# charles-kmc/Semi-blind-image-deblurring-problems-with-TV

Hardware: AMD Instinct MI355X
Metric: SALSA outer-iters/sec + final PSNR, 2048x2048 Gaussian blur (higher is better)
Workload: dtype f64; 1 GPU; SALSA_v2 TV deblur, one 2048x2048 image per GPU, Gaussian PSF 7x7, BSNR 30 dB, TViters=10; images_per_gpu=1, parallelism=images x1

## Files before the change

semi-blind-image-deblurring-problems-with-tv_amd/csrc/ctx.hip:

```cpp
#include <chrono>
#include <cmath>
#include <cstring>
#include <algorithm>
#include <mutex>
#include <thread>
#include <vector>

#include "sbtv_internal.h"

namespace sbtv {

static std::string g_error;
static std::mutex g_error_mu;

void set_global_error(const std::string &msg) {
    std::lock_guard<std::mutex> lk(g_error_mu);
    g_error = msg;
}

int fail(sbtv_ctx *ctx, int code, const std::string &msg) {
    if (ctx) ctx->err = msg;
    set_global_error(msg);
    return code;
}
// ... 348 lines not shown
    const int rc = init();
    if (rc != 0) {
        const std::string msg = ctx->err;
        (void)sbtv_ctx_destroy(ctx);
        return fail(nullptr, rc, msg);
    }
    *out = ctx;
    return 0;
}

int sbtv_ctx_destroy(sbtv_ctx *ctx) {
    if (!ctx) return 0;
    if (ctx->lanes) (void)sbtv_group_destroy(ctx->lanes);
    ctx->lanes = nullptr;
    (void)hipSetDevice(ctx->device);
    if (ctx->stream) (void)hipStreamSynchronize(ctx->stream);
    for (auto &kv : ctx->ws)
        if (kv.second.base) (void)hipFree(kv.second.base);
    if (ctx->canary_desc) (void)hipFree(ctx->canary_desc);
    if (ctx->canary_bad) (void)hipFree(ctx->canary_bad);
    for (auto &kv : ctx->twiddles) (void)hipFree(kv.second);
    for (auto &kv : ctx->any_axes) (void)hipFree(kv.second);
    if (ctx->pinned) (void)hipHostFree(ctx->pinned);
    for (auto &l : ctx->stage) {
        for (int k = 0; k < 2; ++k) {
            if (l.pin[k]) (void)hipHostFree(l.pin[k]);
            if (l.ev[k]) (void)hipEventDestroy(l.ev[k]);
        }
        if (l.s) (void)hipStreamDestroy(l.s);
    }
    for (auto &ev : ctx->ev)
        if (ev) (void)hipEventDestroy(ev);
    for (auto &ev : ctx->loop_ev)
        if (ev) (void)hipEventDestroy(ev);
    if (ctx->own_stream && ctx->stream) (void)hipStreamDestroy(ctx->stream);
    delete ctx;
    return 0;
}

int sbtv_ctx_set_stream(sbtv_ctx *ctx, void *hip_stream) {
    if (!ctx) return SBTV_ERR_BADARG;
    SBTV_HIP(ctx, hipSetDevice(ctx->device));
    SBTV_HIP(ctx, hipStreamSynchronize(ctx->stream));
    if (hip_stream == nullptr) {
        if (!ctx->own_stream) {
            SBTV_HIP(ctx, hipStreamCreateWithFlags(&ctx->stream, hipStreamNonBlocking));
            ctx->own_stream = true;
        }
        return 0;
    }
    if (ctx->own_stream && ctx->stream) SBTV_HIP(ctx, hipStreamDestroy(ctx->stream));
    ctx->stream = (hipStream_t)hip_stream;
    ctx->own_stream = false;
    return 0;
}

int sbtv_ctx_sync(sbtv_ctx *ctx) {
    if (!ctx) return SBTV_ERR_BADARG;
    SBTV_HIP(ctx, hipStreamSynchronize(ctx->stream));
    return 0;
}

int sbtv_callcounter_get(const sbtv_ctx *ctx, long long *calls) {
    if (!ctx || !calls) return SBTV_ERR_BADARG;
    *calls = ctx->calls;
    return 0;
}

int sbtv_callcounter_reset(sbtv_ctx *ctx) {
    if (!ctx) return SBTV_ERR_BADARG;
    ctx->calls = 0;
    return 0;
}

int sbtv_last_timing(const sbtv_ctx *ctx, double out[4]) {
    if (!ctx || !out) return SBTV_ERR_BADARG;
    for (int i = 0; i < 4; ++i) out[i] = ctx->timing[i];
    return 0;
}

int sbtv_last_host_stats(const sbtv_ctx *ctx, double out[14]) {
    if (!ctx || !out) return SBTV_ERR_BADARG;
    const HostStats &h = ctx->hstat;
    const double v[14] = {h.waits, h.ready_at_once, h.waits_slept, h.sleeps, h.stream_queries,
                          h.wait_s, h.wait_max_s, h.enqueue_s, h.enqueue_max_s, h.wait_max_outer,
                          h.nvcsw, h.nivcsw, h.minflt, h.majflt};
    for (int i = 0; i < 14; ++i) out[i] = v[i];
    return 0;
}

int sbtv_host_transpose(const double *src, double *dst, int batch, int rows, int cols) {
    if (!src || !dst || batch < 0 || rows < 0 || cols < 0) return SBTV_ERR_BADARG;
    constexpr int BS = 64;
    const long long nbr = ((long long)rows + BS - 1) / BS;
    const long long jobs = nbr * batch;
    auto work = [&](int t, int T) {
        for (long long job = t; job < jobs; job += T) {
            const int b = (int)(job / nbr), r0 = (int)(job % nbr) * BS, r1 = std::min(rows, r0 + BS);
            const double *s = src + (size_t)b * rows * cols;
            double *d = dst + (size_t)b * rows * cols;
            for (int c0 = 0; c0 < cols; c0 += BS) {
                const int c1 = std::min(cols, c0 + BS);
                for (int c = c0; c < c1; ++c)
                    for (int r = r0; r < r1; ++r) d[(size_t)c * rows + r] = s[(size_t)r * cols + c];
            }
        }
    };
    const size_t bytes = (size_t)batch * rows * cols * sizeof(double);
    const int T = bytes >= ((size_t)4 << 20) ? 4 : 1;
    std::vector<std::thread> th;
    int started = 1;
    try {
        for (int t = 1; t < T; ++t, ++started) th.emplace_back(work, t, T);
    } catch (...) {
    }
    work(0, T);
    for (auto &x : th) x.join();
    for (int t = started; t < T; ++t) work(t, T);
    return 0;
}

int sbtv_diag_solve_stats(const sbtv_ctx *ctx, double out[4]) {
    if (!ctx || !out) return SBTV_ERR_BADARG;
    for (int i = 0; i < 4; ++i) out[i] = ctx->solve_stats[i];
    if (ctx->lanes)
        for (int r = 0; r < sbtv_group_size(ctx->lanes); ++r)
            for (int i = 0; i < 4; ++i) out[i] += sbtv_group_ctx(ctx->lanes, r)->solve_stats[i];
    return 0;
}

int sbtv_diag_stage_stats(const sbtv_ctx *ctx, double out[4]) {
    if (!ctx || !out) return SBTV_ERR_BADARG;
    for (int i = 0; i < 4; ++i) out[i] = ctx->stage_stats[i];
    if (ctx->lanes)
        for (int r = 0; r < sbtv_group_size(ctx->lanes); ++r)
            for (int i = 0; i < 4; ++i) out[i] += sbtv_group_ctx(ctx->lanes, r)->stage_stats[i];
    return 0;
}

int sbtv_diag_workspace(sbtv_ctx *ctx, const char *name, void **dptr, size_t *bytes) {
    if (!ctx || !name || !dptr) return SBTV_ERR_BADARG;
    auto it = ctx->ws.find(name);
    if (it == ctx->ws.end() || !it->second.p) return fail(ctx, SBTV_ERR_BADARG, std::string("no workspace named '") + name + "'");
    *dptr = it->second.p;
    if (bytes) *bytes = it->second.bytes;
    return 0;
}

int sbtv_diag_switches(char *buf, size_t cap) {
    static const char *const names[] = {
        "SBTV_CANARY", "SBTV_COLLECT_RIDE", "SBTV_EXACT", "SBTV_FFT_WAVE", "SBTV_FISTA_FUSED_STEP", "SBTV_FISTA_LAG",
        "SBTV_FUSED_VARIANT", "SBTV_GRAPH", "SBTV_INLINE_CTRL", "SBTV_PROX_SPEC", "SBTV_SAPG_DEFER",
        "SBTV_SAPG_FUSED_MYULA", "SBTV_SAPG_HOST", "SBTV_SINGLE_STEP", "SBTV_SPIN", "SBTV_TAG_SPIN_US", "SBTV_TILE_ORDER", "SBTV_SALSA_NOX", "SBTV_CSALSA_SPECTRAL",
        "SBTV_CORAL_BATCH", "SBTV_ROWS_FOLD", "SBTV_ERR_SUBSET", "SBTV_LANES", "SBTV_LANE_COUNT", "SBTV_STAGE_THREADS", "SBTV_TEST_FAIL_SAPG", "SBTV_FUSED_STAGGER"};
    if (!buf || cap == 0) return SBTV_ERR_BADARG;
    std::string s;
    int nset = 0;
    for (const char *n : names)
        if (const char *e = getenv(n)) {
            s += (nset++ ? " " : "");
            s += n;
            s += "=";
            s += e;
        }
    if (s.size() + 1 > cap) s.resize(cap - 1);
    memcpy(buf, s.c_str(), s.size() + 1);
    return nset;
}

int sbtv_diag_canary(sbtv_ctx *ctx, int poke, int *enabled, int *nbuf, int *nbad) {
    if (!ctx) return SBTV_ERR_BADARG;
    SBTV_HIP(ctx, hipSetDevice(ctx->device));
    if (enabled) *enabled = ctx->canary ? 1 : 0;
    int nb = 0, bad = 0;
    if (ctx->canary && poke) {
        for (auto &kv : ctx->ws)
            if (kv.second.base) {
                SBTV_HIP(ctx, hipMemsetAsync(static_cast<unsigned char *>(kv.second.p) + kv.second.bytes, 0, 8, ctx->stream));
                break;
            }
    }
    std::string name;
    SBTV_TRY(canary_verify(ctx, &nb, &bad, &name));
    if (ctx->canary && poke && bad) {
        for (auto &kv : ctx->ws)
            if (kv.second.base) {
                SBTV_HIP(ctx, hipMemsetAsync(static_cast<unsigned char *>(kv.second.p) + kv.second.bytes, kGuardByte, kGuard, ctx->stream));
                break;
            }
        SBTV_HIP(ctx, hipStreamSynchronize(ctx->stream));
    }
    if (nbuf) *nbuf = nb;
    if (nbad) *nbad = bad;
    return 0;
}

int sbtv_malloc(sbtv_ctx *ctx, size_t bytes, void **dptr) {
    if (!ctx || !dptr) return SBTV_ERR_BADARG;
    SBTV_HIP(ctx, hipSetDevice(ctx->device));
    SBTV_HIP(ctx, hipMalloc(dptr, bytes));
    return 0;
}

int sbtv_free(sbtv_ctx *ctx, void *dptr) {
    if (!ctx) return SBTV_ERR_BADARG;
    SBTV_HIP(ctx, hipStreamSynchronize(ctx->stream));
    SBTV_HIP(ctx, hipFree(dptr));
    return 0;
}

int sbtv_memcpy_h2d(sbtv_ctx *ctx, void *dst, const void *src, size_t bytes) {
    if (!ctx) return SBTV_ERR_BADARG;
    SBTV_HIP(ctx, hipSetDevice(ctx->device));
    if (stage_threaded(bytes)) {
        SBTV_HIP(ctx, hipStreamSynchronize(ctx->stream));
        return stage_copy(ctx, dst, src, bytes, true);
    }
    SBTV_HIP(ctx, hipMemcpyAsync(dst, src, bytes, hipMemcpyHostToDevice, ctx->stream));
    SBTV_HIP(ctx, hipStreamSynchronize(ctx->stream));
    return 0;
}

int sbtv_memcpy_d2h(sbtv_ctx *ctx, void *dst, const void *src, size_t bytes) {
    if (!ctx) return SBTV_ERR_BADARG;
    SBTV_HIP(ctx, hipSetDevice(ctx->device));
    if (stage_threaded(bytes)) {
        SBTV_HIP(ctx, hipStreamSynchronize(ctx->stream));
        return stage_copy(ctx, dst, src, bytes, false);
    }
    SBTV_HIP(ctx, hipMemcpyAsync(dst, src, bytes, hipMemcpyDeviceToHost, ctx->stream));
    SBTV_HIP(ctx, hipStreamSynchronize(ctx->stream));
    return 0;
}

static double spectral_norm_sq(const double *D, int t) {
    double B[15 * 15];
    for (int i = 0; i < t; ++i)
        for (int j = 0; j < t; ++j) {
            double s = 0.0;
            for (int k = 0; k < t; ++k) s += D[i * t + k] * D[j * t + k];
            B[i * t + j] = s;
        }
    for (int sweep = 0; sweep < 60; ++sweep) {
        double off = 0.0, diag = 0.0;
        for (int i = 0; i < t; ++i)
            for (int j = 0; j < t; ++j) (i == j ? diag : off) += B[i * t + j] * B[i * t + j];
        if (off <= 1e-34 * diag || off == 0.0) break;
        for (int p = 0; p < t - 1; ++p)
            for (int q = p + 1; q < t; ++q) {
                const double apq = B[p * t + q];
                if (apq == 0.0) continue;
                const double theta = (B[q * t + q] - B[p * t + p]) / (2.0 * apq);
                const double tt = (theta >= 0 ? 1.0 : -1.0) / (fabs(theta) + sqrt(theta * theta + 1.0));
                const double cs = 1.0 / sqrt(tt * tt + 1.0), sn = tt * cs;
                for (int k = 0; k < t; ++k) {
                    const double bkp = B[k * t + p], bkq = B[k * t + q];
                    B[k * t + p] = cs * bkp - sn * bkq;
                    B[k * t + q] = sn * bkp + cs * bkq;
                }
                for (int k = 0; k < t; ++k) {
                    const double bpk = B[p * t + k], bqk = B[q * t + k];
                    B[p * t + k] = cs * bpk - sn * bqk;
                    B[q * t + k] = sn * bpk + cs * bqk;
                }
            }
    }
    double mx = 0.0;
    for (int i = 0; i < t; ++i) mx = fmax(mx, B[i * t + i]);
    return mx;
}

int sbtv_err_psf(int kind, int taille, const double *ps, int n, const double *p_true, double phi, double *out) {
    if (kind < 0 || kind > 2 || taille < 1 || taille > 15 || !ps || !p_true || !out || n < 1)
        return fail(nullptr, SBTV_ERR_PSF, "sbtv_err_psf: bad arguments");
    const int t2 = taille * taille;
    double truth[225], cur[225], D[225];
    double pt[3] = {p_true[0], kind == SBTV_PSF_LAPLACE ? 0.0 : p_true[1], kind == SBTV_PSF_GAUSSIAN ? phi : 0.0};
    int rc = sbtv_psf_taps(kind, taille, pt, truth, nullptr, nullptr);
    if (rc != 0) return rc;
    for (int i = 0; i < n; ++i) {
        if (kind == SBTV_PSF_MOFFAT && i == 0) {
            out[0] = 0.0;
            continue;
        }
        double p[3] = {ps[i], 0.0, kind == SBTV_PSF_GAUSSIAN ? phi : 0.0};
        if (kind == SBTV_PSF_GAUSSIAN) p[1] = ps[n + (i > 0 ? i - 1 : 0)];
        if (kind == SBTV_PSF_MOFFAT) p[1] = ps[n + i];
        rc = sbtv_psf_taps(kind, taille, p, cur, nullptr, nullptr);
        if (rc != 0) return rc;
        for (int q = 0; q < t2; ++q) D[q] = cur[q] - truth[q];
        out[i] = spectral_norm_sq(D, taille);
    }
    return 0;
}

int sbtv_psf_taps(int kind, int taille, const double *p, double *taps, double *d0, double *d1) {
    if (taille < 1 || taille > 15 || !p || !taps)
        return fail(nullptr, SBTV_ERR_PSF, "sbtv_psf_taps: bad arguments (1 <= taille <= 15)");
    const int t = taille;
    if (kind != SBTV_PSF_GAUSSIAN && kind != SBTV_PSF_MOFFAT && kind != SBTV_PSF_LAPLACE)
        return fail(nullptr, SBTV_ERR_PSF, "sbtv_psf_taps: unknown PSF kind");
    std::vector<double> f(t * t), e0(t * t, 0.0), e1(t * t, 0.0);
    double s = 0, s0 = 0, s1 = 0;
    for (int q = 0; q < t * t; ++q) psf_taps_point(kind, t, p, q, &f[q], &e0[q], &e1[q]);
    for (int q = 0; q < t * t; ++q) { s += f[q]; s0 += e0[q]; s1 += e1[q]; }
    for (int q = 0; q < t * t; ++q) {
        taps[q] = f[q] / s;
// ... 8 lines not shown
```

semi-blind-image-deblurring-problems-with-tv_amd/csrc/elementwise.hip:

```cpp
#include "sbtv_internal.h"

#pragma clang fp contract(off)

namespace sbtv {

constexpr int EWB = 256;

__device__ __forceinline__ double ew_wave_sum(double v) {
#pragma unroll
    for (int off = 32; off > 0; off >>= 1) v += __shfl_xor(v, off, 64);
    return v;
}

template <int NQ>
__device__ __forceinline__ void ew_block_sum(double (&v)[NQ], double *red ) {
    const int lane = threadIdx.x & 63, w = threadIdx.x >> 6;
#pragma unroll
    for (int c = 0; c < NQ; ++c) {
        const double a = ew_wave_sum(v[c]);
        if (lane == 0) red[c * 4 + w] = a;
    }
    __syncthreads();
    if (threadIdx.x == 0) {
#pragma unroll
        for (int c = 0; c < NQ; ++c) v[c] = (red[c * 4] + red[c * 4 + 1]) + (red[c * 4 + 2] + red[c * 4 + 3]);
    }
}

int ew_blocks(size_t P) {
    size_t nb = (P / 2 + EWB - 1) / EWB;
    if (nb > 1024) nb = 1024;
    if (nb < 1) nb = 1;
    return (int)nb;
}

__global__ __launch_bounds__(EWB) void salsa_zero_start_kernel(const double *__restrict__ y, const double *__restrict__ tru,
                                                                double *__restrict__ x, double *__restrict__ u,
                                                                double *__restrict__ bu, double *__restrict__ accp,
                                                                double *__restrict__ postp, size_t P, double scale) {
    const int b = blockIdx.y;
    __shared__ double red[2 * 4];
    const size_t base = (size_t)b * P;
    double acc[2] = {0, 0};
    for (size_t q = (size_t)blockIdx.x * EWB + threadIdx.x; q < P; q += (size_t)gridDim.x * EWB) {
        const double yv = y[base + q];
        const double tv = tru ? tru[base + q] : 0.0;
        acc[0] += yv * yv;
        acc[1] += tv * tv;
        x[base + q] = 0.0;
        u[base + q] = 0.0;
        bu[base + q] = 0.0;
    }
    ew_block_sum<2>(acc, red);
    if (threadIdx.x == 0) {
        const size_t G = gridDim.x;
        for (int q = 0; q < 3; ++q) accp[((size_t)b * 3 + q) * G + blockIdx.x] = (q == 0) ? acc[0] * scale : 0.0;
        for (int q = 0; q < 6; ++q) postp[((size_t)b * 6 + q) * G + blockIdx.x] = (q == 0) ? acc[1] : 0.0;
    }
}

__global__ __launch_bounds__(EWB) void pair_sums_kernel(const double *__restrict__ a, const double *__restrict__ c,
                                                         double *__restrict__ partials, size_t P) {
    const int b = blockIdx.y;
    __shared__ double red[3 * 4];
    __shared__ double redm[4];
    const size_t base = (size_t)b * P;
    double acc[3] = {0, 0, 0};
    double mx = -1.0e308;
    for (size_t q = (size_t)blockIdx.x * EWB + threadIdx.x; q < P; q += (size_t)gridDim.x * EWB) {
        const double av = a[base + q];
        const double cv = c ? c[base + q] : 0.0;
        const double d = av - cv;
        acc[0] += d * d;
        acc[1] += av * av;
        acc[2] += cv * cv;
        mx = fmax(mx, av);
    }
    for (int off = 32; off > 0; off >>= 1) mx = fmax(mx, __shfl_xor(mx, off, 64));
    if ((threadIdx.x & 63) == 0) redm[threadIdx.x >> 6] = mx;
    ew_block_sum<3>(acc, red);
    if (threadIdx.x == 0) {
        for (int q = 0; q < 3; ++q) partials[((size_t)b * 4 + q) * gridDim.x + blockIdx.x] = acc[q];
        partials[((size_t)b * 4 + 3) * gridDim.x + blockIdx.x] = fmax(fmax(redm[0], redm[1]), fmax(redm[2], redm[3]));
    }
}

__global__ __launch_bounds__(256) void reduce_max_kernel(const double *__restrict__ partials, int n,
                                                          double *__restrict__ out) {
    __shared__ double redm[4];
    const double *p = partials + (size_t)blockIdx.x * n;
    double mx = -1.0e308;
    for (int q = threadIdx.x; q < n; q += 256) mx = fmax(mx, p[q]);
    for (int off = 32; off > 0; off >>= 1) mx = fmax(mx, __shfl_xor(mx, off, 64));
    if ((threadIdx.x & 63) == 0) redm[threadIdx.x >> 6] = mx;
    __syncthreads();
    if (threadIdx.x == 0) out[blockIdx.x] = fmax(fmax(redm[0], redm[1]), fmax(redm[2], redm[3]));
}

__global__ __launch_bounds__(EWB) void axpy_kernel(double *__restrict__ y, const double *__restrict__ gr, double a,
                                                    size_t Ptot, ProxArm arm, int batch) {
    if (arm.ctrl && blockIdx.x == 0 && (int)threadIdx.x < batch) {
        const int b = threadIdx.x;
        ProxCtrl c = arm.ctrl[b];
        c.k = 0;
        c.done = (arm.frozen && arm.frozen[b]) ? 1 : 0;
        c.cur = 0;
        c.maxiter = arm.maxiter;
        c.redo = 0;
        c.f_valid = 0;
        c.err = 0.0;
        c.lambda = arm.lambda[b];
        c.tol = arm.tol;
        c.tau = arm.tau;
        arm.ctrl[b] = c;
    }
    for (size_t q = (size_t)blockIdx.x * EWB + threadIdx.x; q < Ptot / 2; q += (size_t)gridDim.x * EWB) {
        double2 yv = *reinterpret_cast<double2 *>(y + 2 * q);
        const double2 gv = *reinterpret_cast<const double2 *>(gr + 2 * q);
        yv.x = yv.x - a * gv.x;
        yv.y = yv.y - a * gv.y;
        *reinterpret_cast<double2 *>(y + 2 * q) = yv;
    }
}
__global__ __launch_bounds__(EWB) void fista_momentum_kernel(const double *__restrict__ x, const double *__restrict__ xold,
                                                              double *__restrict__ y, const double *__restrict__ tru,
                                                              double c, double *__restrict__ partials, size_t P,
                                                              const int *__restrict__ frozen) {
    const int b = blockIdx.y;
    if (frozen && frozen[b]) return;
    __shared__ double red[3 * 4];
    const size_t base = (size_t)b * P;
    double acc[3] = {0, 0, 0};
    for (size_t q = (size_t)blockIdx.x * EWB + threadIdx.x; q < P / 2; q += (size_t)gridDim.x * EWB) {
        const size_t o = base + 2 * q;
        const double2 xv = *reinterpret_cast<const double2 *>(x + o);
        const double2 xo = *reinterpret_cast<const double2 *>(xold + o);
        const double d0 = xv.x - xo.x, d1 = xv.y - xo.y;
        *reinterpret_cast<double2 *>(y + o) = make_double2(xv.x + c * d0, xv.y + c * d1);
        if (tru) {
            const double2 tv = *reinterpret_cast<const double2 *>(tru + o);
            const double e0 = xv.x - tv.x, e1 = xv.y - tv.y;
            acc[0] += e0 * e0 + e1 * e1;
        }
        acc[1] += d0 * d0 + d1 * d1;
        acc[2] += xv.x * xv.x + xv.y * xv.y;
    }
    ew_block_sum<3>(acc, red);
    if (threadIdx.x == 0)
        for (int q = 0; q < 3; ++q) partials[((size_t)b * 3 + q) * gridDim.x + blockIdx.x] = acc[q];
}

template <bool MOM>
__global__ __launch_bounds__(EWB) void myula_step_kernel(double *__restrict__ X, const double *__restrict__ prox,
                                                          const double *__restrict__ grad,
                                                          const double *__restrict__ Z,
                                                          const double *__restrict__ sigma2, double gam, double lamb,
                                                          double sq2g, size_t P, RngArgs rng, ProxArm arm, MomArgs mom) {
    const int b = blockIdx.y;
    if (arm.ctrl && blockIdx.x == 0 && threadIdx.x == 0) {
        ProxCtrl c = arm.ctrl[b];
        c.k = 0;
        c.done = 0;
        c.cur = 0;
        c.maxiter = arm.maxiter;
        c.redo = 0;
        c.f_valid = 0;
        c.err = 0.0;
        c.lambda = arm.lambda[b];
        c.tol = arm.tol;
        c.tau = arm.tau;
        arm.ctrl[b] = c;
    }
    const size_t base = (size_t)b * P;
    const double s2 = sigma2[b];
    const unsigned step = rng.step_dev ? (unsigned)rng.step_dev[0] : rng.step;
    const int k = MOM ? mom_sample(mom) : 0;
    const double rk = 1.0 / (double)(k > 0 ? k : 1);
    for (size_t q = (size_t)blockIdx.x * EWB + threadIdx.x; q < P / 2; q += (size_t)gridDim.x * EWB) {
        const size_t o = base + 2 * q;
        const double2 xv = *reinterpret_cast<const double2 *>(X + o);
        const double2 pv = *reinterpret_cast<const double2 *>(prox + o);
        const double2 gv = *reinterpret_cast<const double2 *>(grad + o);
        const double2 zv = Z ? *reinterpret_cast<const double2 *>(Z + o)
                             : philox_normal_pair(q, step, rng.chain0 + (unsigned)b, rng.seed);
        double2 r;
        r.x = myula_nocontract(xv.x, pv.x, gv.x, 1.0, zv.x, gam, lamb, s2, sq2g);
        r.y = myula_nocontract(xv.y, pv.y, gv.y, 1.0, zv.y, gam, lamb, s2, sq2g);
        *reinterpret_cast<double2 *>(X + o) = r;
        if (MOM && k > 0) moments_pair(mom, o, r, k, rk);
    }
}

template <bool MOM>
__global__ __launch_bounds__(EWB) void myula_plain_kernel(double *__restrict__ X, const double *__restrict__ prox,
                                                           const double *__restrict__ grad,
                                                           const double *__restrict__ Z,
                                                           const double *__restrict__ sigma2, double gam, double lamb,
                                                           double sq2g, size_t P, RngArgs rng, ProxArm arm, MomArgs mom) {
    const int b = blockIdx.y;
    if (arm.ctrl && blockIdx.x == 0 && threadIdx.x == 0) {
        ProxCtrl c = arm.ctrl[b];
        c.k = 0;
        c.done = 0;
        c.cur = 0;
        c.maxiter = arm.maxiter;
        c.redo = 0;
        c.f_valid = 0;
        c.err = 0.0;
        c.lambda = arm.lambda[b];
        c.tol = arm.tol;
        c.tau = arm.tau;
        arm.ctrl[b] = c;
    }
    const size_t base = (size_t)b * P;
    const double s2 = sigma2[b], keep = 1.0 - gam / lamb;
    const int k = MOM ? mom_sample(mom) : 0;
    const double rk = 1.0 / (double)(k > 0 ? k : 1);
    for (size_t q = (size_t)blockIdx.x * EWB + threadIdx.x; q < P / 2; q += (size_t)gridDim.x * EWB) {
        const size_t o = base + 2 * q;
        const double2 xv = *reinterpret_cast<const double2 *>(X + o);
        const double2 pv = *reinterpret_cast<const double2 *>(prox + o);
        const double2 gv = *reinterpret_cast<const double2 *>(grad + o);
        const double2 zv = Z ? *reinterpret_cast<const double2 *>(Z + o)
                             : philox_normal_pair(q, rng.step, rng.chain0 + (unsigned)b, rng.seed);
        double2 r;
        r.x = (keep * xv.x - gam * (gv.x / s2 - pv.x / lamb)) + sq2g * zv.x;
        r.y = (keep * xv.y - gam * (gv.y / s2 - pv.y / lamb)) + sq2g * zv.y;
        *reinterpret_cast<double2 *>(X + o) = r;
        if (MOM && k > 0) moments_pair(mom, o, r, k, rk);
    }
}

__global__ __launch_bounds__(EWB) void moments_seed_kernel(const double *__restrict__ X, double *__restrict__ mean,
                                                           double *__restrict__ m2, size_t n2) {
    const MomArgs m{mean, m2, 1, nullptr, 1, 1};
    for (size_t q = (size_t)blockIdx.x * EWB + threadIdx.x; q < n2; q += (size_t)gridDim.x * EWB)
        moments_pair(m, 2 * q, *reinterpret_cast<const double2 *>(X + 2 * q), 1, 1.0);
}

__global__ __launch_bounds__(EWB) void moments_finish_kernel(const double *__restrict__ mean, const double *__restrict__ m2,
                                                             size_t P, int batch, double n, int pooled, int raw,
                                                             double *__restrict__ mean_out, double *__restrict__ var_out) {
#pragma clang fp contract(off)
    const int b = blockIdx.y;
    for (size_t i = (size_t)blockIdx.x * EWB + threadIdx.x; i < P; i += (size_t)gridDim.x * EWB) {
        double mu = mean[(size_t)b * P + i], s = m2[(size_t)b * P + i], na = n;
        if (pooled) {
            for (int c = 1; c < batch; ++c) {
                const double mb = mean[(size_t)c * P + i], sb = m2[(size_t)c * P + i];
                const double nt = na + n, d = mb - mu;
                mu = mu + d * (n / nt);
                s = (s + sb) + d * d * (na * n / nt);
                na = nt;
            }
        }
        mean_out[(size_t)b * P + i] = mu;
        if (var_out) var_out[(size_t)b * P + i] = raw ? s : (na > 1.0 ? s / (na - 1.0) : 0.0);
    }
}

int myula_plain_step(sbtv_ctx *ctx, double *X, const double *prox, const double *grad, const double *Z,
                     const double *sigma2_dev, double gam, double lamb, size_t P, int batch, const RngArgs *rng,
                     const ProxArm *arm, const MomArgs *mom) {
    if (!Z && !rng) return fail(ctx, SBTV_ERR_BADARG, "myula_plain_step: neither a noise array nor generator arguments");
    const RngArgs r = rng ? *rng : RngArgs{0ull, 0u, 0u, nullptr};
    const ProxArm pa = arm ? *arm : ProxArm{nullptr, nullptr, 0, 0.0, 0.0, nullptr};
    if (mom)
        hipLaunchKernelGGL(myula_plain_kernel<true>, dim3(ew_blocks(P), batch), dim3(EWB), 0, ctx->stream, X, prox, grad, Z,
                           sigma2_dev, gam, lamb, sqrt(2 * gam), P, r, pa, *mom);
    else
        hipLaunchKernelGGL(myula_plain_kernel<false>, dim3(ew_blocks(P), batch), dim3(EWB), 0, ctx->stream, X, prox, grad, Z,
                           sigma2_dev, gam, lamb, sqrt(2 * gam), P, r, pa, MomArgs{});
    SBTV_HIP(ctx, hipGetLastError());
    return 0;
}

int moments_seed(sbtv_ctx *ctx, const double *X, double *mean, double *m2, size_t P, int batch) {
    const size_t n = P * batch;
    hipLaunchKernelGGL(moments_seed_kernel, dim3(ew_blocks(n)), dim3(EWB), 0, ctx->stream, X, mean, m2, n / 2);
    SBTV_HIP(ctx, hipGetLastError());
    return 0;
}

int moments_finish(sbtv_ctx *ctx, const double *mean, const double *m2, size_t P, int batch, long long n, const MomReq &req) {
    const int pooled = req.pooled && !req.raw;
    const size_t nout = P * (pooled ? 1 : batch);
    double *mo = nullptr, *vo = nullptr;
    const int fl = req.dev ? SBTV_DEVICE_PTRS : SBTV_HOST_PTRS;
    SBTV_TRY(stage_out_buf(ctx, "mom.mean_out", req.mean, nout, fl, &mo));
    if (req.var) SBTV_TRY(stage_out_buf(ctx, "mom.var_out", req.var, nout, fl, &vo));
    hipLaunchKernelGGL(moments_finish_kernel, dim3(ew_blocks(2 * P), pooled ? 1 : batch), dim3(EWB), 0, ctx->stream, mean,
                       m2, P, batch, (double)n, pooled, req.raw ? 1 : 0, mo, vo);
    SBTV_HIP(ctx, hipGetLastError());
    SBTV_TRY(stage_out_copy(ctx, req.mean, mo, nout, fl));
    if (req.var) SBTV_TRY(stage_out_copy(ctx, req.var, vo, nout, fl));
    if (req.count)
        for (size_t c = 0; c < (pooled ? 1 : (size_t)batch); ++c) req.count[c] = pooled ? n * batch : n;
    return 0;
}

int pair_sums(sbtv_ctx *ctx, const double *a, const double *c, size_t P, int batch, double *out4_dev) {
    const int nb = ew_blocks(P);
    double *partials = nullptr;
    SBTV_TRY(ws_get_t(ctx, "ew.pair.partials", (size_t)batch * 4 * nb, &partials));
    hipLaunchKernelGGL(pair_sums_kernel, dim3(nb, batch), dim3(EWB), 0, ctx->stream, a, c, partials, P);
    SBTV_HIP(ctx, hipGetLastError());
    for (int b = 0; b < batch; ++b) {
        SBTV_TRY(reduce_partials(ctx, partials + (size_t)b * 4 * nb, 3, nb, out4_dev + (size_t)b * 4));
        hipLaunchKernelGGL(reduce_max_kernel, dim3(1), dim3(256), 0, ctx->stream, partials + ((size_t)b * 4 + 3) * nb,
                           nb, out4_dev + (size_t)b * 4 + 3);
    }
    SBTV_HIP(ctx, hipGetLastError());
    return 0;
}

int salsa_zero_start(sbtv_ctx *ctx, const double *y, const double *tru, double *x, double *u, double *bu, size_t P, int batch,
                     double scale, double **accp, double **postp, int *nblk) {
    const int G = ew_blocks(2 * P);
    SBTV_TRY(ws_get_t(ctx, "ew.zero.acc", (size_t)batch * 3 * G, accp));
    SBTV_TRY(ws_get_t(ctx, "ew.zero.post", (size_t)batch * 6 * G, postp));
    hipLaunchKernelGGL(salsa_zero_start_kernel, dim3(G, batch), dim3(EWB), 0, ctx->stream, y, tru, x, u, bu, *accp, *postp, P,
                       scale);
    SBTV_HIP(ctx, hipGetLastError());
    *nblk = G;
    return 0;
}

int axpy(sbtv_ctx *ctx, double *y, const double *gr, double a, size_t Ptot, const ProxArm *arm, int batch) {
    if (arm && batch > EWB) return fail(ctx, SBTV_ERR_BADARG, "axpy: cannot arm more than 256 control blocks");
    const ProxArm pa = arm ? *arm : ProxArm{nullptr, nullptr, 0, 0.0, 0.0, nullptr};
    hipLaunchKernelGGL(axpy_kernel, dim3(ew_blocks(Ptot)), dim3(EWB), 0, ctx->stream, y, gr, a, Ptot, pa, batch);
    SBTV_HIP(ctx, hipGetLastError());
    return 0;
}

int fista_momentum(sbtv_ctx *ctx, const double *x, const double *xold, double *y, const double *tru, double coef,
                   double *partials, size_t P, int batch, const int *frozen) {
    hipLaunchKernelGGL(fista_momentum_kernel, dim3(ew_blocks(P), batch), dim3(EWB), 0, ctx->stream, x, xold, y, tru,
                       coef, partials, P, frozen);
    SBTV_HIP(ctx, hipGetLastError());
    return 0;
}

int myula_step(sbtv_ctx *ctx, double *X, const double *prox, const double *grad, const double *Z,
               const double *sigma2_dev, double gam, double lamb, size_t P, int batch, const RngArgs *rng,
               const ProxArm *arm, const MomArgs *mom) {
    if (!Z && !rng) return fail(ctx, SBTV_ERR_BADARG, "myula_step: neither a noise array nor generator arguments");
    const RngArgs r = rng ? *rng : RngArgs{0ull, 0u, 0u, nullptr};
    const ProxArm pa = arm ? *arm : ProxArm{nullptr, nullptr, 0, 0.0, 0.0, nullptr};
    if (mom)
        hipLaunchKernelGGL(myula_step_kernel<true>, dim3(ew_blocks(P), batch), dim3(EWB), 0, ctx->stream, X, prox, grad, Z,
                           sigma2_dev, gam, lamb, sqrt(2 * gam), P, r, pa, *mom);
    else
        hipLaunchKernelGGL(myula_step_kernel<false>, dim3(ew_blocks(P), batch), dim3(EWB), 0, ctx->stream, X, prox, grad, Z,
                           sigma2_dev, gam, lamb, sqrt(2 * gam), P, r, pa, MomArgs{});
    SBTV_HIP(ctx, hipGetLastError());
    return 0;
}

}

using namespace sbtv;

extern "C" {

static int metric_common(sbtv_ctx *ctx, const double *x_true, const double *x, int M, int N, int batch, double *out,
                         int flags, bool psnr) {
    if (!ctx) return SBTV_ERR_BADARG;
    if (!x_true || !x || !out || M < 1 || N < 1 || batch < 1) return fail(ctx, SBTV_ERR_BADARG, "metric: bad arguments");
    SBTV_HIP(ctx, hipSetDevice(ctx->device));
    const size_t P = (size_t)M * N;
    const double *a = nullptr, *c = nullptr;
    SBTV_TRY(stage_in(ctx, "metric.a", x_true, P * batch, flags, &a));
    SBTV_TRY(stage_in(ctx, "metric.c", x, P * batch, flags, &c));
    double *o4 = nullptr;
    SBTV_TRY(ws_get_t(ctx, "metric.out", (size_t)batch * 4, &o4));
    SBTV_TRY(pair_sums(ctx, a, c, P, batch, o4));
    std::vector<double> h((size_t)batch * 4);
    SBTV_HIP(ctx, hipMemcpyAsync(h.data(), o4, sizeof(double) * batch * 4, hipMemcpyDeviceToHost, ctx->stream));
    SBTV_HIP(ctx, hipStreamSynchronize(ctx->stream));
    for (int b = 0; b < batch; ++b) {
        const double se = h[(size_t)b * 4], mx = h[(size_t)b * 4 + 3];
        if (psnr)
            out[b] = 10 * log10(mx * mx) - 10 * log10(se / (double)P);
        else
            out[b] = 10 * log10(se / (double)P);
    }
    return canary_epilogue(ctx, 0);
}

int sbtv_PSNR(sbtv_ctx *ctx, const double *x_true, const double *x, int M, int N, int batch, double *out, int flags) {
    return metric_common(ctx, x_true, x, M, N, batch, out, flags, true);
}
int sbtv_MSE(sbtv_ctx *ctx, const double *x_true, const double *x, int M, int N, int batch, double *out, int flags) {
    return metric_common(ctx, x_true, x, M, N, batch, out, flags, false);
}

}
```

semi-blind-image-deblurring-problems-with-tv_amd/csrc/fft.hip:

```cpp
#include <type_traits>

#include "sbtv_internal.h"

namespace sbtv {

__device__ __forceinline__ double2 cadd(double2 a, double2 b) { return make_double2(a.x + b.x, a.y + b.y); }
__device__ __forceinline__ double2 csub(double2 a, double2 b) { return make_double2(a.x - b.x, a.y - b.y); }
__device__ __forceinline__ double2 cmul(double2 a, double2 b) {
    return make_double2(a.x * b.x - a.y * b.y, a.x * b.y + a.y * b.x);
}
__device__ __forceinline__ double2 cmulc(double2 a, double2 b) {
    return make_double2(a.x * b.x + a.y * b.y, a.y * b.x - a.x * b.y);
}
__device__ __forceinline__ double2 cconj(double2 a) { return make_double2(a.x, -a.y); }
__device__ __forceinline__ double2 cscale(double2 a, double s) { return make_double2(a.x * s, a.y * s); }
__device__ __forceinline__ double cabs2(double2 a) { return a.x * a.x + a.y * a.y; }

constexpr int TWS = 2;
constexpr int TW = 1 << TWS;
__device__ __forceinline__ size_t s_tiled(int k, int l, int n1) {
    return (((size_t)(l >> TWS) * n1 + k) << TWS) + (l & (TW - 1));
}
__device__ __forceinline__ size_t u_tiled(int k, int l, int n1) { return ((size_t)(l >> TWS) * (n1 + 1) + k) * TW + (l & (TW - 1)); }

// ... 264 lines not shown
        double2 r;
        if (e == 0) {
            r = make_double2(Z.x + Z.y, Z.x - Z.y);
        } else {
            const double2 w = tw_M[e];
            const double2 su = cadd(Z, Zm), di = csub(Z, Zm);
            const double2 wd = cmul(w, di);
            r = make_double2(0.5 * (su.x + wd.y), 0.5 * (su.y - wd.x));
        }
        out[e] = r;
    }
}

typedef double sbtv_d2 __attribute__((ext_vector_type(2)));
__device__ __forceinline__ double2 nt_load2(const double *p) {
    const sbtv_d2 v = __builtin_nontemporal_load(reinterpret_cast<const sbtv_d2 *>(p));
    return make_double2(v.x, v.y);
}
__device__ __forceinline__ void nt_store2(double *p, double2 v) {
    sbtv_d2 w;
    w.x = v.x;
    w.y = v.y;
    __builtin_nontemporal_store(w, reinterpret_cast<sbtv_d2 *>(p));
}
template <int LOG2N, bool POST>
__global__ __launch_bounds__(COLS_THREADS) void fft_cols_inv_kernel(const double2 *__restrict__ S,
                                                                     double *__restrict__ x,
                                                                     const double2 *__restrict__ tw_n1,
                                                                     const double2 *__restrict__ tw_M, int N,
                                                                     double scale, const int *__restrict__ frozen,
                                                                     ColsPost post) {
    constexpr int n = 1 << LOG2N, T = n / 8;
    constexpr int LDSN = n + (n >> 3);
    constexpr int MAXSEQ = (COLS_THREADS / T) > 0 ? (COLS_THREADS / T) : 1;
    __shared__ double lds[2 * MAXSEQ * LDSN];
    const int b = blockIdx.y;
    if (frozen && frozen[b]) return;
    const int nseq = blockDim.x / T;
    const int seq = threadIdx.x / T, t = threadIdx.x - seq * T;
    const int j = blockIdx.x * nseq + seq;
    const size_t colbase = ((size_t)b * N + j) * n;
    const double2 *__restrict__ in = S + colbase;
    ColsX X{lds + seq * LDSN, MAXSEQ * LDSN};
    double2 v[8], m[8];
#pragma unroll
    for (int s = 0; s < 8; ++s) v[s] = in[t + s * T];
    constexpr bool PREP = POST && (LOG2N <= 8);
    double2 pu[PREP ? 8 : 1], pb[PREP ? 8 : 1], pt[PREP ? 8 : 1], pul[PREP ? 8 : 1], pxo[PREP ? 8 : 1];
    double pup[PREP ? 8 : 1];
    if constexpr (PREP) {
        constexpr int M = 2 * n;
        const size_t ibase = (size_t)b * N * M, cb = ibase + (size_t)j * M;
        const size_t cl = ibase + (size_t)(j > 0 ? j - 1 : N - 1) * M;
#pragma unroll
        for (int s = 0; s < 8; ++s) {
            const int e = t + s * T;
            const size_t o = cb + 2 * (size_t)e;
            pu[s] = *reinterpret_cast<const double2 *>(post.u + o);
            pb[s] = *reinterpret_cast<const double2 *>(post.bu + o);
            if (post.tru) pt[s] = nt_load2(post.tru + o);
            if (post.xprev) pxo[s] = *reinterpret_cast<const double2 *>(post.xprev + o);
            pup[s] = post.u[e > 0 ? o - 1 : cb + M - 1];
            pul[s] = *reinterpret_cast<const double2 *>(post.u + cl + 2 * (size_t)e);
        }
    }
    mirror<LOG2N>(v, m, t, X);
#pragma unroll
    for (int s = 0; s < 8; ++s) {
        const int e = t + s * T;
        if (e == 0) {
            const double X0 = v[s].x, Xn = v[s].y;
            v[s] = make_double2(0.5 * (X0 + Xn), 0.5 * (X0 - Xn));
        } else {
            const double2 Xk = v[s], Xm = cconj(m[s]);
            const double2 E = cscale(cadd(Xk, Xm), 0.5);
            const double2 O = cmulc(cscale(csub(Xk, Xm), 0.5), tw_M[e]);
            v[s] = make_double2(E.x - O.y, E.y + O.x);
        }
    }
    fft_stages<LOG2N, 0, true>(v, t, tw_n1, X);
    double2 *__restrict__ out = reinterpret_cast<double2 *>(x) + colbase;
    if constexpr (!POST) {
#pragma unroll
        for (int s = 0; s < 8; ++s) out[t + s * T] = cscale(v[s], scale);
    } else {
        constexpr int M = 2 * n;
        const size_t ibase = (size_t)b * N * M;
        const size_t cb = ibase + (size_t)j * M;
        const size_t cl = ibase + (size_t)(j > 0 ? j - 1 : N - 1) * M;
        double acc[6] = {0.0, 0.0, 0.0, 0.0, 0.0, 0.0};
#pragma unroll
        for (int s = 0; s < 8; ++s) {
            const int e = t + s * T;
            const size_t o = cb + 2 * (size_t)e;
            const double2 xv = cscale(v[s], scale);
            nt_store2(reinterpret_cast<double *>(out + e), xv);
            const double2 uv = PREP ? pu[PREP ? s : 0] : *reinterpret_cast<const double2 *>(post.u + o);
            double2 bv = PREP ? pb[PREP ? s : 0] : *reinterpret_cast<const double2 *>(post.bu + o);
            bv.x = bv.x + (uv.x - xv.x);
            bv.y = bv.y + (uv.y - xv.y);
            *reinterpret_cast<double2 *>(post.bu + o) = bv;
            *reinterpret_cast<double2 *>(post.g + o) = make_double2(xv.x - bv.x, xv.y - bv.y);
            if (post.tru) {
                const double2 tv = PREP ? pt[PREP ? s : 0] : nt_load2(post.tru + o);
                const double e0 = xv.x - tv.x, e1 = xv.y - tv.y;
                acc[0] += e0 * e0 + e1 * e1;
            }
            const double d0 = xv.x - uv.x, d1 = xv.y - uv.y;
            acc[1] += d0 * d0 + d1 * d1;
            acc[2] += xv.x * xv.x + xv.y * xv.y;
            acc[3] += uv.x * uv.x + uv.y * uv.y;
            if (post.xprev) {
                const double2 xo = PREP ? pxo[PREP ? s : 0] : *reinterpret_cast<const double2 *>(post.xprev + o);
                const double p0 = xv.x - xo.x, p1 = xv.y - xo.y;
                acc[4] += p0 * p0 + p1 * p1;
            }
            const double up = PREP ? pup[PREP ? s : 0] : post.u[e > 0 ? o - 1 : cb + M - 1];
            const double2 ul = PREP ? pul[PREP ? s : 0] : *reinterpret_cast<const double2 *>(post.u + cl + 2 * (size_t)e);
            const double h0 = uv.x - ul.x, v0 = uv.x - up, h1 = uv.y - ul.y, v1 = uv.y - uv.x;
            acc[5] += sqrt(h0 * h0 + v0 * v0) + sqrt(h1 * h1 + v1 * v1);
        }
        __syncthreads();
        const int nthr = blockDim.x;
#pragma unroll
        for (int c = 0; c < 6; ++c) lds[c * nthr + threadIdx.x] = acc[c];
        __syncthreads();
        for (int stride = nthr >> 1; stride > 0; stride >>= 1) {
            if ((int)threadIdx.x < stride) {
#pragma unroll
                for (int c = 0; c < 6; ++c) lds[c * nthr + threadIdx.x] += lds[c * nthr + threadIdx.x + stride];
            }
            __syncthreads();
        }
        if (threadIdx.x < 6) post.partials[((size_t)b * 6 + threadIdx.x) * gridDim.x + blockIdx.x] = lds[threadIdx.x * nthr];
    }
}

struct RowsParams {
    const double2 *Sin;
    double2 *Sout;
    const double2 *tw;
    const double2 *H, *Y, *D1, *D2;
    double2 *E;
    const double *cs;
    const double *mu;
    double *acc;
    const int *frozen;
    int n1;
    int fwd, inv, op;
    int shared_spec;
    int fold;
    size_t u_img;
    int u_tiled;
};

template <int OP>
__device__ __forceinline__ double2 spec_apply(double2 V, double2 H, double2 Y, double2 D1, double2 D2, double mu,
                                              double wgt, double (&acc)[3]) {
    if constexpr (OP == OP_MUL_H) {
        return cmul(V, H);
    } else if constexpr (OP == OP_MUL_HC) {
        return cmulc(V, H);
    } else if constexpr (OP == OP_INVLS) {
        const double d = cabs2(H) + mu;
        return make_double2(V.x / d, V.y / d);
    } else if constexpr (OP == OP_ATA) {
        return cscale(V, cabs2(H));
    } else if constexpr (OP == OP_SALSA) {
        const double d = cabs2(H) + mu;
        const double2 num = cadd(cmulc(Y, H), cscale(V, mu));
#ifdef SBTV_SPEC_IEEE_DIV
        const double rd = 1.0 / d;
#else
        const double rd = fast_rcp(d);
#endif
        const double2 Xh = make_double2(num.x * rd, num.y * rd);
        const double2 R = csub(Y, cmul(H, Xh));
        acc[0] += wgt * cabs2(R);
        return Xh;
    } else if constexpr (OP == OP_RESID) {
        const double2 R = csub(cmul(H, V), Y);
        acc[0] += wgt * cabs2(R);
        return V;
    } else if constexpr (OP == OP_GRADF) {
        const double2 R = csub(cmul(H, V), Y);
        acc[0] += wgt * cabs2(R);
        return cmulc(R, H);
    } else if constexpr (OP == OP_GRAD) {
        const double2 R = csub(cmul(H, V), Y);
        acc[0] += wgt * cabs2(R);
        const double2 d1 = cmulc(cmul(D1, V), R), d2 = cmulc(cmul(D2, V), R);
        acc[1] += wgt * d1.x;
        acc[2] += wgt * d2.x;
        return cmulc(R, H);
    } else {
        return V;
    }
}

struct CsPar {
    double c_y, c_e, c_keep;
};
__device__ __forceinline__ double2 spec_apply_cs(double2 V, double2 H, double2 Y, double2 &E, double mu, const CsPar &c,
                                                 double wgt, double (&acc)[3]) {
    const double d = cabs2(H) + mu;
    const double2 W = cadd(cscale(Y, c.c_y), cscale(E, c.c_e));
    const double2 num = cadd(cmulc(W, H), cscale(V, mu));
#ifdef SBTV_SPEC_IEEE_DIV
    const double rd = 1.0 / d;
#else
    const double rd = fast_rcp(d);
#endif
    const double2 Xh = make_double2(num.x * rd, num.y * rd);
    const double2 T = csub(cmul(H, Xh), Y);
    const double2 En = cadd(T, cscale(E, c.c_keep));
    acc[0] += wgt * cabs2(T);
    acc[1] += wgt * cabs2(En);
    acc[2] += wgt * cabs2(csub(En, E));
    E = En;
    return Xh;
}

template <int LOG2N, int RK, int OP>
__global__ __launch_bounds__(RK *((1 << LOG2N) / 8), 1) void fft_rows_kernel(RowsParams p) {
    constexpr int N = 1 << LOG2N, T = N / 8;
    constexpr int LDSI = RK * N;
    constexpr int LDSN = LDSI + ((LDSI >> 5) << 2) + 8;
    __shared__ double lds[2 * LDSN];
    __shared__ double red[3 * 16];
    const int b = blockIdx.y;
    if (p.frozen && p.frozen[b]) return;
    const int q = threadIdx.x % RK, t = threadIdx.x / RK;
    int kb;
    {
        const int nt = gridDim.x, bid = blockIdx.x;
        const int q8 = nt >> 3, r8 = nt & 7, x = bid & 7, o = bid >> 3;
        kb = (x < r8 ? x * (q8 + 1) : r8 * (q8 + 1) + (x - r8) * q8) + o;
    }
    const int k = kb * RK + q;
    const int n1 = p.n1;
    const size_t ibase = (size_t)b * n1 * N;
    const double2 *__restrict__ in = p.Sin + ibase;
    RowsX<RK> X{lds, LDSN, q};
    double2 v[8];
    auto sidx = [&](int l) -> size_t { return (size_t)l * n1 + k; };
    auto uidx = [&](int kk, int l) -> size_t { return (size_t)l * (p.n1 + 1) + kk; };
#pragma unroll
    for (int s = 0; s < 8; ++s) v[s] = in[sidx(t + s * T)];
    constexpr bool CS = (OP == OP_CSALSA);
    constexpr bool PRE = (OP != OP_NONE) && !CS && (RK * T <= 256);
    constexpr bool needY = (OP == OP_SALSA || OP == OP_RESID || OP == OP_GRAD || OP == OP_GRADF || CS);
    constexpr bool needD = (OP == OP_GRAD);
    const size_t hbase = p.shared_spec ? 0 : (size_t)b * p.u_img;
    double2 hh[PRE ? 8 : 1], yy[(PRE && needY) ? 8 : 1], dd1[(PRE && needD) ? 8 : 1], dd2[(PRE && needD) ? 8 : 1];
    double2 hq[PRE ? 8 : 1], yq[(PRE && needY) ? 8 : 1], d1q[(PRE && needD) ? 8 : 1], d2q[(PRE && needD) ? 8 : 1];
    if constexpr (PRE) {
#pragma unroll
        for (int s = 0; s < 8; ++s) {
            const size_t hi = hbase + uidx(k, t + s * T);
            hh[s] = p.H[hi];
            if constexpr (needY) yy[s] = p.Y[hi];
            if constexpr (needD) {
                dd1[s] = p.D1[hi];
                dd2[s] = p.D2[hi];
            }
        }
        if (kb == 0 && q == 0) {
#pragma unroll
            for (int s = 0; s < 8; ++s) {
                const size_t hn = hbase + uidx(n1, t + s * T);
                hq[s] = p.H[hn];
                if constexpr (needY) yq[s] = p.Y[hn];
                if constexpr (needD) {
                    d1q[s] = p.D1[hn];
                    d2q[s] = p.D2[hn];
                }
            }
        }
    }
    if (p.fwd) fft_stages<LOG2N, 0, false>(v, t, p.tw, X);

    double acc[3] = {0.0, 0.0, 0.0};
    if constexpr (OP != OP_NONE) {
        const double mu = p.mu ? p.mu[b] : 0.0;
        if constexpr (CS) {
            const CsPar cp{p.cs[0], p.cs[1], p.cs[2]};
            double2 *__restrict__ Ep = p.E + hbase;
            const double2 *__restrict__ Hp = p.H + hbase, *__restrict__ Yp = p.Y + hbase;
            if (kb == 0) {
                double2 m[8];
                mirror<LOG2N>(v, m, t, X);
#pragma unroll
                for (int s = 0; s < 8; ++s) {
                    const int l = t + s * T;
                    if (q == 0) {
                        const size_t h0 = uidx(0, l), hn = uidx(n1, l);
                        const double2 P = v[s], Q = cconj(m[s]);
                        const double2 A = cscale(cadd(P, Q), 0.5);
                        const double2 dB = csub(P, Q);
                        const double2 B = make_double2(0.5 * dB.y, -0.5 * dB.x);
                        double2 e0 = Ep[h0], en = Ep[hn];
                        const double2 A2 = spec_apply_cs(A, Hp[h0], Yp[h0], e0, mu, cp, 1.0, acc);
                        const double2 B2 = spec_apply_cs(B, Hp[hn], Yp[hn], en, mu, cp, 1.0, acc);
                        Ep[h0] = e0;
                        Ep[hn] = en;
                        v[s] = make_double2(A2.x - B2.y, A2.y + B2.x);
// ... 261 lines not shown
    const PassDims cd = cols_dims(pl);
    hipLaunchKernelGGL((fft_cols_inv_kernel<L, false>), dim3(cd.wgs, pl.batch), dim3(cd.threads), 0,
                       ctx->stream, S, x, pl.tw_n1, pl.tw_M, pl.N, scale, frozen, ColsPost{});
}
template <int L>
static void launch_cols_inv_post(sbtv_ctx *ctx, const FftPlan &pl, const double2 *S, double *x, double scale,
                                 const int *frozen, const ColsPost &post) {
    const PassDims cd = cols_dims(pl);
    hipLaunchKernelGGL((fft_cols_inv_kernel<L, true>), dim3(cd.wgs, pl.batch), dim3(cd.threads), 0,
                       ctx->stream, S, x, pl.tw_n1, pl.tw_M, pl.N, scale, frozen, post);
}

#define SBTV_DISPATCH_LOG2(L, CALL)                                    \
    switch (L) {                                                       \
        case 3: CALL(3); break;                                        \
        case 4: CALL(4); break;                                        \
        case 5: CALL(5); break;                                        \
        case 6: CALL(6); break;                                        \
        case 7: CALL(7); break;                                        \
        case 8: CALL(8); break;                                        \
        case 9: CALL(9); break;                                        \
        case 10: CALL(10); break;                                      \
        case 11: CALL(11); break;                                      \
        default: return fail(ctx, SBTV_ERR_SIZE, "unsupported FFT length"); \
    }

bool fft_cols_tv_ok(const FftPlan &pl) { return !pl.generic; }
int fft_cols_fwd_f(sbtv_ctx *ctx, const FftPlan &pl, const double *x, const double *add, double2 *S,
                   const int *frozen, double *tvp) {
    if (tvp && (!fft_cols_tv_ok(pl) || add)) return fail(ctx, SBTV_ERR_BADARG, "fft_cols_fwd: TV partials not available for this call");
    if (pl.generic) return any_cols_fwd(ctx, pl, x, add, S, frozen);
    if (pl.wave) {
        const PassDims cd = cols_dims(pl);
        const dim3 grid(cd.wgs, pl.batch), block(cd.threads);
        if (pl.n1 == 1024)
            hipLaunchKernelGGL((cols_fwd_wave_kernel<10, 16>), grid, block, 0, ctx->stream, x, add, S, pl.tw_n1, pl.tw_M,
                               pl.N, frozen, tvp);
        else
            hipLaunchKernelGGL((cols_fwd_wave_kernel<9, 8>), grid, block, 0, ctx->stream, x, add, S, pl.tw_n1, pl.tw_M,
                               pl.N, frozen, tvp);
        SBTV_HIP(ctx, hipGetLastError());
        return 0;
    }
    const int L = ilog2(pl.n1);
#define CALL(LL) launch_cols_fwd<LL>(ctx, pl, x, add, S, frozen, tvp)
    SBTV_DISPATCH_LOG2(L, CALL)
#undef CALL
    SBTV_HIP(ctx, hipGetLastError());
    return 0;
}
int fft_cols_fwd(sbtv_ctx *ctx, const FftPlan &pl, const double *x, const double *add, double2 *S) {
    return fft_cols_fwd_f(ctx, pl, x, add, S, nullptr, nullptr);
}

int fft_cols_inv_f(sbtv_ctx *ctx, const FftPlan &pl, const double2 *S, double *x, double scale, const int *frozen) {
    if (pl.generic) return any_cols_inv(ctx, pl, S, x, scale, frozen, nullptr);
    if (pl.wave) {
        const PassDims cd = cols_dims(pl);
        const dim3 grid(cd.wgs, pl.batch), block(cd.threads);
        if (pl.n1 == 1024)
            hipLaunchKernelGGL((cols_inv_wave_kernel<10, 16, 0>), grid, block, 0, ctx->stream, S, x, pl.tw_n1,
                               pl.tw_M, pl.N, scale, frozen, ColsPost{});
        else
            hipLaunchKernelGGL((cols_inv_wave_kernel<9, 8, 0>), grid, block, 0, ctx->stream, S, x, pl.tw_n1, pl.tw_M,
                               pl.N, scale, frozen, ColsPost{});
        SBTV_HIP(ctx, hipGetLastError());
        return 0;
    }
    const int L = ilog2(pl.n1);
#define CALL(LL) launch_cols_inv<LL>(ctx, pl, S, x, scale, frozen)
    SBTV_DISPATCH_LOG2(L, CALL)
#undef CALL
    SBTV_HIP(ctx, hipGetLastError());
    return 0;
}
bool fft_cols_inv_step_ok(const FftPlan &pl) { return !pl.generic && pl.wave; }
static int fft_cols_step_check(sbtv_ctx *ctx, const FftPlan &pl, const char *who) {
    if (!fft_cols_inv_step_ok(pl)) return fail(ctx, SBTV_ERR_BADARG, std::string(who) + ": size not on the wave-granular path");
    return 0;
}
int fft_cols_inv_step(sbtv_ctx *ctx, const FftPlan &pl, const double2 *S, double *y, double scale, double alpha,
                      const int *frozen) {
    SBTV_TRY(fft_cols_step_check(ctx, pl, "fft_cols_inv_step"));
    ColsPost post;
    post.ystep = y;
    post.alpha = alpha;
    const PassDims cd = cols_dims(pl);
        const dim3 grid(cd.wgs, pl.batch), block(cd.threads);
    if (pl.n1 == 1024)
        hipLaunchKernelGGL((cols_inv_wave_kernel<10, 16, 8>), grid, block, 0, ctx->stream, S, (double *)nullptr, pl.tw_n1,
                           pl.tw_M, pl.N, scale, frozen, post);
    else
        hipLaunchKernelGGL((cols_inv_wave_kernel<9, 8, 8>), grid, block, 0, ctx->stream, S, (double *)nullptr, pl.tw_n1, pl.tw_M,
                           pl.N, scale, frozen, post);
    SBTV_HIP(ctx, hipGetLastError());
    return 0;
}
int fft_cols_inv_sub(sbtv_ctx *ctx, const FftPlan &pl, const double2 *S, double *x, double scale, const double *b, double *g) {
    SBTV_TRY(fft_cols_step_check(ctx, pl, "fft_cols_inv_sub"));
    ColsPost post;
    post.bu_in = b;
    post.g = g;
    const PassDims cd = cols_dims(pl);
        const dim3 grid(cd.wgs, pl.batch), block(cd.threads);
    if (pl.n1 == 1024)
        hipLaunchKernelGGL((cols_inv_wave_kernel<10, 16, 64>), grid, block, 0, ctx->stream, S, x, pl.tw_n1, pl.tw_M, pl.N, scale,
                           (const int *)nullptr, post);
    else
        hipLaunchKernelGGL((cols_inv_wave_kernel<9, 8, 64>), grid, block, 0, ctx->stream, S, x, pl.tw_n1, pl.tw_M, pl.N, scale,
                           (const int *)nullptr, post);
    SBTV_HIP(ctx, hipGetLastError());
    return 0;
}
int fft_cols_inv_myula(sbtv_ctx *ctx, const FftPlan &pl, const double2 *S, double scale, double *X, const double *prox,
                       const double *Z, const double *sigma2_dev, double gam, double lamb, const RngArgs *rng,
                       const ProxArm *arm, const MomArgs *mom) {
    SBTV_TRY(fft_cols_step_check(ctx, pl, "fft_cols_inv_myula"));
    if (!Z && !rng) return fail(ctx, SBTV_ERR_BADARG, "fft_cols_inv_myula: neither a noise array nor generator arguments");
    ColsPost post;
    post.ystep = X;
    post.mprox = prox;
    post.mZ = Z;
    post.msig2 = sigma2_dev;
    post.mgam = gam;
    post.mlamb = lamb;
    post.msq2g = sqrt(2 * gam);
    if (rng) post.mrng = *rng;
    if (arm) post.marm = *arm;
    const PassDims cd = cols_dims(pl);
        const dim3 grid(cd.wgs, pl.batch), block(cd.threads);
    if (mom) {
        post.mom = *mom;
        if (pl.n1 == 1024)
            hipLaunchKernelGGL((cols_inv_wave_kernel<10, 16, 16 | 128>), grid, block, 0, ctx->stream, S, (double *)nullptr,
                               pl.tw_n1, pl.tw_M, pl.N, scale, (const int *)nullptr, post);
        else
            hipLaunchKernelGGL((cols_inv_wave_kernel<9, 8, 16 | 128>), grid, block, 0, ctx->stream, S, (double *)nullptr,
                               pl.tw_n1, pl.tw_M, pl.N, scale, (const int *)nullptr, post);
    } else if (pl.n1 == 1024)
        hipLaunchKernelGGL((cols_inv_wave_kernel<10, 16, 16>), grid, block, 0, ctx->stream, S, (double *)nullptr, pl.tw_n1,
                           pl.tw_M, pl.N, scale, (const int *)nullptr, post);
    else
        hipLaunchKernelGGL((cols_inv_wave_kernel<9, 8, 16>), grid, block, 0, ctx->stream, S, (double *)nullptr, pl.tw_n1, pl.tw_M,
                           pl.N, scale, (const int *)nullptr, post);
    SBTV_HIP(ctx, hipGetLastError());
    return 0;
}
int fft_cols_inv(sbtv_ctx *ctx, const FftPlan &pl, const double2 *S, double *x, double scale) {
    return fft_cols_inv_f(ctx, pl, S, x, scale, nullptr);
}
int fft_cols_blocks(const FftPlan &pl) { return (pl.wave || pl.generic) ? pl.N : pl.N / cols_nseq(pl); }
int fft_cols_inv_post(sbtv_ctx *ctx, const FftPlan &pl, const double2 *S, double *x, double scale, const int *frozen,
                      const ColsPost &post) {
    if ((!pl.wave && (post.bu_in || post.skip_x)) || (post.bu_in && !post.skip_x))
        return fail(ctx, SBTV_ERR_BADARG, "fft_cols_inv_post: bu_in + skip_x go together and need the wave-granular column pass");
    if (pl.generic) return any_cols_inv(ctx, pl, S, x, scale, frozen, &post);
    if (pl.wave) {
        const PassDims cd = cols_dims(pl);
        const dim3 grid(cd.wgs, pl.batch), block(cd.threads);
        if (post.skip_x && (!post.bu_in || post.bu_in == post.bu || post.xprev))
            return fail(ctx, SBTV_ERR_BADARG, "fft_cols_inv_post: skip_x needs a separate bu_in and no xprev");
        const int pm = 1 + (post.tru ? 2 : 0) + (post.xprev ? 4 : 0) + (post.skip_x ? 32 : 0);
#define SBTV_POST_CASE(PM_)                                                                                          \
    case PM_:                                                                                                        \
        if (pl.n1 == 1024)                                                                                           \
            hipLaunchKernelGGL((cols_inv_wave_kernel<10, 16, PM_>), grid, block, 0, ctx->stream, S, x, pl.tw_n1,       \
                               pl.tw_M, pl.N, scale, frozen, post);                                                  \
        else                                                                                                         \
            hipLaunchKernelGGL((cols_inv_wave_kernel<9, 8, PM_>), grid, block, 0, ctx->stream, S, x, pl.tw_n1,         \
                               pl.tw_M, pl.N, scale, frozen, post);                                                  \
        break;
        switch (pm) {
            SBTV_POST_CASE(1)
            SBTV_POST_CASE(3)
            SBTV_POST_CASE(5)
            SBTV_POST_CASE(7)
            SBTV_POST_CASE(33)
            SBTV_POST_CASE(35)
        }
#undef SBTV_POST_CASE
        SBTV_HIP(ctx, hipGetLastError());
        return 0;
    }
    const int L = ilog2(pl.n1);
#define CALL(LL) launch_cols_inv_post<LL>(ctx, pl, S, x, scale, frozen, post)
    SBTV_DISPATCH_LOG2(L, CALL)
#undef CALL
    SBTV_HIP(ctx, hipGetLastError());
    return 0;
}

static inline int rows_rk(const FftPlan &pl) {
    const int N = pl.N;
    if (N == 4096) return 2;
    const int rk = (N >= 512) ? 4 : 8;
    const int small = (N == 512) ? 1 : (N == 256) ? 2 : rk;
    return (pl.n1 / rk < 128) ? small : rk;
}
static inline PassDims rows_dims(const FftPlan &pl) {
    if (pl.generic) return {0, ANY_SPEC_THREADS, ANY_SPEC_BLOCKS};
    if (pl.wave) return {4, pl.N / 4, pl.n1 / 4};
    const int rk = rows_rk(pl);
    return {rk, rk * (pl.N / 8), pl.n1 / rk};
}
bool fft_rows_csalsa_ok(const FftPlan &pl) { return !pl.generic; }
static int fft_rows_check(sbtv_ctx *ctx, const FftPlan &pl, int op) {
    if (op == OP_CSALSA && !fft_rows_csalsa_ok(pl)) return fail(ctx, SBTV_ERR_SIZE, "row pass: OP_CSALSA is not built for this plan");
    return 0;
}
int fft_rows_blocks(const FftPlan &pl) {
    return rows_dims(pl).wgs;
}

static inline bool rows_fold_ok(const FftPlan &pl, int shared_spec) {
    static const bool fold_wanted = [] {
        const char *e = getenv("SBTV_ROWS_FOLD");
        return !(e && e[0] == '0');
    }();
    return fold_wanted && pl.wave && shared_spec && pl.batch > 1 && ((pl.n1 / 4) % 8 == 0);
}
template <int L>
static void launch_rows_pipe(sbtv_ctx *ctx, const FftPlan &pl, const RowsParams &p0) {
    RowsParams p = p0;
    const bool fold = rows_fold_ok(pl, p.shared_spec);
    p.fold = fold ? pl.batch : 0;
    const PassDims rd = rows_dims(pl);
    const dim3 grid(fold ? rd.wgs * pl.batch : rd.wgs, fold ? 1 : pl.batch), block(rd.threads);
#define SBTV_ROWS_OP(OP_)                                                                                     \
    case OP_: hipLaunchKernelGGL((rows_pipe_kernel<L, OP_>), grid, block, 0, ctx->stream, p); break;
    switch (p.op) {
        SBTV_ROWS_OP(OP_NONE)
        SBTV_ROWS_OP(OP_MUL_H)
        SBTV_ROWS_OP(OP_MUL_HC)
        SBTV_ROWS_OP(OP_INVLS)
        SBTV_ROWS_OP(OP_SALSA)
        SBTV_ROWS_OP(OP_RESID)
        SBTV_ROWS_OP(OP_GRAD)
        SBTV_ROWS_OP(OP_ATA)
        SBTV_ROWS_OP(OP_GRADF)
        SBTV_ROWS_OP(OP_CSALSA)
        default: break;
    }
#undef SBTV_ROWS_OP
}

template <int L, int RK>
static void launch_rows(sbtv_ctx *ctx, const FftPlan &pl, const RowsParams &p) {
    const PassDims rd = rows_dims(pl);
    const dim3 grid(rd.wgs, pl.batch), block(rd.threads);
#define SBTV_ROWS_OP(OP_)                                                                                     \
    case OP_: hipLaunchKernelGGL((fft_rows_kernel<L, RK, OP_>), grid, block, 0, ctx->stream, p); break;
    switch (p.op) {
        SBTV_ROWS_OP(OP_NONE)
        SBTV_ROWS_OP(OP_MUL_H)
        SBTV_ROWS_OP(OP_MUL_HC)
        SBTV_ROWS_OP(OP_INVLS)
        SBTV_ROWS_OP(OP_SALSA)
        SBTV_ROWS_OP(OP_RESID)
        SBTV_ROWS_OP(OP_GRAD)
        SBTV_ROWS_OP(OP_ATA)
        SBTV_ROWS_OP(OP_GRADF)
        SBTV_ROWS_OP(OP_CSALSA)
        default: break;
    }
#undef SBTV_ROWS_OP
}

int fft_rows(sbtv_ctx *ctx, const FftPlan &pl, const double2 *Sin, double2 *Sout, const RowsArgs &a) {
    RowsParams p;
    p.Sin = Sin;
    p.Sout = Sout;
    p.tw = pl.tw_N;
    p.H = a.H;
    p.Y = a.Y;
    p.D1 = a.D1;
    p.D2 = a.D2;
    p.E = a.E;
    p.cs = a.cs;
    p.mu = a.mu;
    p.acc = a.acc;
    p.frozen = a.frozen;
    p.n1 = pl.n1;
    p.fwd = a.dir_fwd;
    p.inv = a.dir_inv;
    p.op = a.op;
    p.shared_spec = a.shared_spec;
    p.fold = 0;
    p.u_img = pl.u_img;
    p.u_tiled = pl.u_tiled;
    SBTV_TRY(fft_rows_check(ctx, pl, a.op));
    if (pl.generic) return any_rows(ctx, pl, p, Sout);
    const int L = ilog2(pl.N);
    if (L > 12) return fail(ctx, SBTV_ERR_SIZE, "row FFT: N must be <= 4096");
    if (pl.wave) {
        if (L == 11) launch_rows_pipe<11>(ctx, pl, p);
        else launch_rows_pipe<10>(ctx, pl, p);
        SBTV_HIP(ctx, hipGetLastError());
        return 0;
    }
    if (pl.N >= 512) {
        switch (L) {
            case 9:
                if (rows_rk(pl) == 1) launch_rows<9, 1>(ctx, pl, p);
                else launch_rows<9, 4>(ctx, pl, p);
                break;
            case 10: launch_rows<10, 4>(ctx, pl, p); break;
            case 11: launch_rows<11, 4>(ctx, pl, p); break;
            case 12: launch_rows<12, 2>(ctx, pl, p); break;
            default: break;
        }
    } else {
        switch (L) {
            case 4: launch_rows<4, 8>(ctx, pl, p); break;
            case 5: launch_rows<5, 8>(ctx, pl, p); break;
            case 6: launch_rows<6, 8>(ctx, pl, p); break;
            case 7: launch_rows<7, 8>(ctx, pl, p); break;
            case 8:
                if (rows_rk(pl) == 2) launch_rows<8, 2>(ctx, pl, p);
                else launch_rows<8, 8>(ctx, pl, p);
                break;
            default: return fail(ctx, SBTV_ERR_SIZE, "row FFT: N must be >= 16");
        }
    }
    SBTV_HIP(ctx, hipGetLastError());
    return 0;
}

int spec_unpack(sbtv_ctx *ctx, const FftPlan &pl, const double2 *S, double2 *U) {
    if (pl.generic) {
        SBTV_HIP(ctx, hipMemcpyAsync(U, S, sizeof(double2) * pl.s_img * pl.batch, hipMemcpyDeviceToDevice, ctx->stream));
        return 0;
    }
    if (pl.wave) {
        hipLaunchKernelGGL(spec_unpack_tiled_kernel, dim3((pl.N + 63) / 64, pl.n1 + 1, pl.batch), dim3(64), 0,
                           ctx->stream, S, U, pl.n1, pl.N, pl.u_tiled);
        SBTV_HIP(ctx, hipGetLastError());
        return 0;
    }
    const int thr = 64;
    hipLaunchKernelGGL(spec_unpack_kernel, dim3((pl.n1 + 1 + thr - 1) / thr, pl.N, pl.batch), dim3(thr), 0,
                       ctx->stream, S, U, pl.n1, pl.N);
    SBTV_HIP(ctx, hipGetLastError());
    return 0;
}

static inline int psf_lch(const FftPlan &pl) {
    const size_t elems = (size_t)(pl.n1 + 1) * pl.N * pl.batch;
    const int lch = (int)(elems >> 19);
    return lch < 1 ? 1 : (lch > 16 ? 16 : lch);
}
int psf_spectrum_sets(sbtv_ctx *ctx, const FftPlan &pl, const double *const *taps_dev, int taille, double2 *const *U, int nsets) {
    const int thr = 64;
    if (taille > PSF_TMAX) return fail(ctx, SBTV_ERR_PSF, "PSF larger than 15 x 15");
    if (nsets < 1 || nsets > 3) return fail(ctx, SBTV_ERR_BADARG, "psf_spectrum_sets: 1..3 tap sets");
    if (pl.generic) {
        for (int q = 0; q < nsets; ++q) SBTV_TRY(any_psf_spectrum(ctx, pl, taps_dev[q], taille, U[q]));
        return 0;
    }
    const int lch = psf_lch(pl);
    PsfSets ps{};
    for (int q = 0; q < 3; ++q) {
        ps.taps[q] = taps_dev[q < nsets ? q : 0];
        ps.U[q] = U[q < nsets ? q : 0];
    }
    const dim3 grid = pl.u_tiled ? dim3(((pl.n1 + 1) * 4 + thr - 1) / thr, ((pl.N >> 2) + lch - 1) / lch, pl.batch * nsets)
                                 : dim3((pl.n1 + 1 + thr - 1) / thr, (pl.N + lch - 1) / lch, pl.batch * nsets);
    if (taille == 7)
        hipLaunchKernelGGL(psf_spectrum_kernel<7>, grid, dim3(thr), 0, ctx->stream, ps, taille, pl.batch, pl.n1, pl.M, pl.N,
                           pl.tw_M, pl.tw_N, lch, pl.u_tiled);
    else
        hipLaunchKernelGGL(psf_spectrum_kernel<0>, grid, dim3(thr), 0, ctx->stream, ps, taille, pl.batch, pl.n1, pl.M, pl.N,
                           pl.tw_M, pl.tw_N, lch, pl.u_tiled);
    SBTV_HIP(ctx, hipGetLastError());
    return 0;
}
int psf_spectrum(sbtv_ctx *ctx, const FftPlan &pl, const double *taps_dev, int taille, double2 *U) {
    return psf_spectrum_sets(ctx, pl, &taps_dev, taille, &U, 1);
}

}

using namespace sbtv;

extern "C" {

int sbtv_rfft2_packed(sbtv_ctx *ctx, const double *in, double *out, int M, int N, int batch, int inverse, int flags) {
    if (!ctx) return SBTV_ERR_BADARG;
    if (!in || !out || batch < 1) return fail(ctx, SBTV_ERR_BADARG, "rfft2_packed: bad arguments");
    SBTV_HIP(ctx, hipSetDevice(ctx->device));
    FftPlan pl;
    SBTV_TRY(fft_plan(ctx, M, N, batch, &pl));
    if (pl.generic)
        return fail(ctx, SBTV_ERR_SIZE, "rfft2_packed: the packed half-spectrum format exists for powers of two 16..4096 only");
    const size_t cnt = (size_t)M * N * batch;
    const double *ind = nullptr;
    double *outd = nullptr;
    SBTV_TRY(stage_in(ctx, "fft.in", in, cnt, flags, &ind));
    SBTV_TRY(stage_out_buf(ctx, "fft.out", out, cnt, flags, &outd));
    double2 *tmp = nullptr;
    SBTV_TRY(ws_get_t(ctx, "fft.tmp", cnt / 2, &tmp));
    RowsArgs a{};
    a.op = OP_NONE;
    double2 *tmp2 = nullptr;
    if (pl.wave) SBTV_TRY(ws_get_t(ctx, "fft.tmp2", cnt / 2, &tmp2));
    auto relayout = [&](const double2 *src, double2 *dst, int to_tiled) -> int {
        hipLaunchKernelGGL(s_relayout_kernel, dim3(1024, batch), dim3(256), 0, ctx->stream, src, dst, pl.n1, N, to_tiled);
        SBTV_HIP(ctx, hipGetLastError());
        return 0;
    };
    if (!inverse) {
        SBTV_TRY(fft_cols_fwd(ctx, pl, ind, nullptr, tmp));
        a.dir_fwd = 1;
        a.dir_inv = 0;
        if (pl.wave) {
            SBTV_TRY(fft_rows(ctx, pl, tmp, tmp2, a));
            SBTV_TRY(relayout(tmp2, reinterpret_cast<double2 *>(outd), 0));
        } else {
            SBTV_TRY(fft_rows(ctx, pl, tmp, reinterpret_cast<double2 *>(outd), a));
        }
    } else {
        a.dir_fwd = 0;
        a.dir_inv = 1;
        if (pl.wave) {
            SBTV_TRY(relayout(reinterpret_cast<const double2 *>(ind), tmp2, 1));
            SBTV_TRY(fft_rows(ctx, pl, tmp2, tmp, a));
        } else {
            SBTV_TRY(fft_rows(ctx, pl, reinterpret_cast<const double2 *>(ind), tmp, a));
        }
        SBTV_TRY(fft_cols_inv(ctx, pl, tmp, outd, 1.0 / ((double)pl.n1 * N)));
    }
    SBTV_TRY(stage_out_copy(ctx, out, outd, cnt, flags));
    if (!(flags & SBTV_DEVICE_PTRS)) SBTV_HIP(ctx, hipStreamSynchronize(ctx->stream));
    return canary_epilogue(ctx, 0);
}

int sbtv_A_wrapper(sbtv_ctx *ctx, const double *taps, int taille, const double *mu, const double *x, double *out,
                   int M, int N, int batch, int mode, int flags) {
    if (!ctx) return SBTV_ERR_BADARG;
    int op;
    switch (mode) {
        case 1: case 3: op = OP_MUL_H; break;
        case 2: op = OP_MUL_HC; break;
        case 9: op = OP_INVLS; break;
// ... 347 lines not shown
```

semi-blind-image-deblurring-problems-with-tv_amd/csrc/fft_wave.inc:

```


struct SyncWave {
    static __device__ __forceinline__ void sync() {
        __builtin_amdgcn_fence(__ATOMIC_RELEASE, "wavefront");
        __builtin_amdgcn_wave_barrier();
        __builtin_amdgcn_fence(__ATOMIC_ACQUIRE, "wavefront");
    }
};
struct SyncBlock {
    static __device__ __forceinline__ void sync() { __syncthreads(); }
};

template <class SYNC>
struct XSeq {
    double2 *buf;
    static __device__ __forceinline__ int idx(int pos) { return pos + (pos >> 4); }
    static __device__ __forceinline__ void sync() { SYNC::sync(); }
};
template <class SYNC>
struct XSwz {
    double2 *buf;
    static __device__ __forceinline__ int idx(int pos) {
        const int m = pos >> 4;
        return pos ^ ((m & 7) ^ ((m & 4) << 1));
// ... 67 lines not shown
    if constexpr (LOG2NS > 0) {
        constexpr int T = (1 << LOG2N) / V;
        constexpr int R = 1 << LR, G = V / R;
        constexpr int SH = LOG2N - LOG2NS - LR;
#pragma unroll
        for (int q = 0; q < G; ++q) {
            const int k = (t + q * T) & ((1 << LOG2NS) - 1);
            if constexpr (R == 16) {
                const double2 w1 = twid<INV>(tw, k << SH), w2 = twid<INV>(tw, (2 * k) << SH);
                const double2 w4 = twid<INV>(tw, (4 * k) << SH), w8 = twid<INV>(tw, (8 * k) << SH);
                const double2 w3 = cmul(w1, w2), w5 = cmul(w1, w4), w6 = cmul(w2, w4), w7 = cmul(w3, w4);
                v[q + 1 * G] = cmul(v[q + 1 * G], w1);
                v[q + 2 * G] = cmul(v[q + 2 * G], w2);
                v[q + 3 * G] = cmul(v[q + 3 * G], w3);
                v[q + 4 * G] = cmul(v[q + 4 * G], w4);
                v[q + 5 * G] = cmul(v[q + 5 * G], w5);
                v[q + 6 * G] = cmul(v[q + 6 * G], w6);
                v[q + 7 * G] = cmul(v[q + 7 * G], w7);
                v[q + 8 * G] = cmul(v[q + 8 * G], w8);
                v[q + 9 * G] = cmul(v[q + 9 * G], cmul(w1, w8));
                v[q + 10 * G] = cmul(v[q + 10 * G], cmul(w2, w8));
                v[q + 11 * G] = cmul(v[q + 11 * G], cmul(w3, w8));
                v[q + 12 * G] = cmul(v[q + 12 * G], cmul(w4, w8));
                v[q + 13 * G] = cmul(v[q + 13 * G], cmul(w5, w8));
                v[q + 14 * G] = cmul(v[q + 14 * G], cmul(w6, w8));
                v[q + 15 * G] = cmul(v[q + 15 * G], cmul(w7, w8));
            } else {
#pragma unroll
                for (int r = 1; r < R; ++r) v[q + r * G] = cmul(v[q + r * G], twid<INV>(tw, (r * k) << SH));
            }
        }
    }
}

template <int V, int LOG2N, int LOG2NS, int LR, class X>
__device__ __forceinline__ void exchange_v(double2 (&v)[V], int t, const X &x) {
    constexpr int T = (1 << LOG2N) / V;
    constexpr int R = 1 << LR, G = V / R;
#pragma unroll
    for (int q = 0; q < G; ++q) {
        const int j = t + q * T;
        const int k = j & ((1 << LOG2NS) - 1);
        const int j0 = ((j >> LOG2NS) << (LOG2NS + LR)) + k;
#pragma unroll
        for (int r = 0; r < R; ++r) x.buf[X::idx(j0 + (r << LOG2NS))] = v[q + r * G];
    }
    X::sync();
#pragma unroll
    for (int s = 0; s < V; ++s) v[s] = x.buf[X::idx(t + s * T)];
    X::sync();
}

template <int V, int LOG2N, int LOG2NS, bool INV, class X, class TW>
__device__ __forceinline__ void stages_v(double2 (&v)[V], int t, TW tw, const X &x) {
    constexpr int left = LOG2N - LOG2NS;
    constexpr int LV = (V == 16) ? 4 : 3;
    if constexpr (left > 0) {
        constexpr int LR = left >= LV ? LV : left;
        twiddles_v<V, LOG2N, LOG2NS, LR, INV>(v, t, tw);
        butterflies_v<V, LR, INV>(v);
        if constexpr (left - LR > 0) {
            exchange_v<V, LOG2N, LOG2NS, LR>(v, t, x);
            stages_v<V, LOG2N, LOG2NS + LR, INV>(v, t, tw, x);
        }
    }
}

template <int LOG2N, int V>
__global__ __launch_bounds__(64 * TW, 2) void cols_fwd_wave_kernel(const double *__restrict__ x,
                                                                 const double *__restrict__ add,
                                                                 double2 *__restrict__ S,
                                                                 const double2 *__restrict__ tw_n1,
                                                                 const double2 *__restrict__ tw_M, int N,
                                                                 const int *__restrict__ frozen,
                                                                 double *__restrict__ tvp) {
    constexpr int n = 1 << LOG2N;
    static_assert(n == 64 * V, "one wave per column");
    constexpr int REG = xseq_elems(n);
    __shared__ __attribute__((aligned(16))) double2 lds[TW * REG];
    const int b = blockIdx.y;
    if (frozen && frozen[b]) return;
    const int w = __builtin_amdgcn_readfirstlane(threadIdx.x >> 6), lane = threadIdx.x & 63;
    const int tile = blockIdx.x;
    const int j = tile * TW + w;
    const size_t colbase = ((size_t)b * N + j) * n;
    const double2 *__restrict__ xin = reinterpret_cast<const double2 *>(x) + colbase;
    XSeq<SyncWave> X{lds + w * REG};
    double2 v[V];
#pragma unroll
    for (int s = 0; s < V; ++s) v[s] = xin[lane + s * 64];
    if (tvp) {
        constexpr int M = 2 * n;
        const double *__restrict__ xl = x + ((size_t)b * N + (j > 0 ? j - 1 : N - 1)) * M;
        double carry = __shfl(v[V - 1].y, 63, 64);
        double a = 0.0;
#pragma unroll
        for (int s = 0; s < V; ++s) {
            const double2 ul = *reinterpret_cast<const double2 *>(xl + 2 * (size_t)(lane + s * 64));
            double upv = __shfl_up(v[s].y, 1, 64);
            if (lane == 0) upv = carry;
            carry = __shfl(v[s].y, 63, 64);
            const double h0 = v[s].x - ul.x, v0 = v[s].x - upv, h1 = v[s].y - ul.y, v1 = v[s].y - v[s].x;
            a += sqrt(h0 * h0 + v0 * v0) + sqrt(h1 * h1 + v1 * v1);
        }
#pragma unroll
        for (int off = 32; off > 0; off >>= 1) a += __shfl_xor(a, off, 64);
        if (lane == 0) tvp[(size_t)b * N + j] = a;
    }
    if (add) {
        const double2 *__restrict__ ain = reinterpret_cast<const double2 *>(add) + colbase;
#pragma unroll
        for (int s = 0; s < V; ++s) v[s] = cadd(v[s], ain[lane + s * 64]);
    }
    stages_v<V, LOG2N, 0, false>(v, lane, tw_n1, X);
    SyncWave::sync();
#pragma unroll
    for (int s = 0; s < V; ++s) X.buf[XSeq<SyncWave>::idx(lane + s * 64)] = v[s];
    __syncthreads();
    double2 *__restrict__ out = S + ((size_t)b * (N >> TWS) + tile) * ((size_t)n << TWS);
#pragma unroll
    for (int i = 0; i < V; ++i) {
        const int flat = i * (64 * TW) + threadIdx.x;
        const int k = flat >> TWS, c = flat & (TW - 1);
        const double2 *reg = lds + c * REG;
        const double2 Z = reg[XSeq<SyncWave>::idx(k)];
        const double2 Zm = cconj(reg[XSeq<SyncWave>::idx((n - k) & (n - 1))]);
        double2 r;
        if (k == 0) {
            r = make_double2(Z.x + Z.y, Z.x - Z.y);
        } else {
            const double2 wv = tw_M[k];
            const double2 su = cadd(Z, Zm), di = csub(Z, Zm);
            const double2 wd = cmul(wv, di);
            r = make_double2(0.5 * (su.x + wd.y), 0.5 * (su.y - wd.x));
        }
        out[flat] = r;
    }
}

__device__ __forceinline__ double2 step_nocontract(double2 y, double a, double2 x) {
#pragma clang fp contract(off)
    const double t0 = a * x.x, t1 = a * x.y;
    return make_double2(y.x - t0, y.y - t1);
}

template <int LOG2N, int V, int PM>
__global__ __launch_bounds__(64 * TW, 2) void cols_inv_wave_kernel(const double2 *__restrict__ S, double *__restrict__ x,
                                                                 const double2 *__restrict__ tw_n1,
                                                                 const double2 *__restrict__ tw_M, int N, double scale,
                                                                 const int *__restrict__ frozen, ColsPost post) {
    constexpr int n = 1 << LOG2N;
    constexpr bool POST = (PM & 1) != 0, HAS_TRU = (PM & 2) != 0, HAS_XPREV = (PM & 4) != 0;
    constexpr bool NOX = (PM & 32) != 0;
    static_assert(n == 64 * V, "one wave per column");
    constexpr int REG = xseq_elems(n);
    __shared__ __attribute__((aligned(16))) double2 lds[TW * REG];
    const int b = blockIdx.y;
    if (frozen && frozen[b]) return;
    const int w = __builtin_amdgcn_readfirstlane(threadIdx.x >> 6), lane = threadIdx.x & 63;
    const int tile = blockIdx.x;
    const int j = tile * TW + w;
    const double2 *__restrict__ in = S + ((size_t)b * (N >> TWS) + tile) * ((size_t)n << TWS);
    {
        double2 a[V];
#pragma unroll
        for (int i = 0; i < V; ++i) a[i] = in[i * (64 * TW) + threadIdx.x];
#pragma unroll
        for (int i = 0; i < V; ++i) {
            const int flat = i * (64 * TW) + threadIdx.x;
            lds[(flat & (TW - 1)) * REG + XSeq<SyncWave>::idx(flat >> TWS)] = a[i];
        }
    }
    __syncthreads();
    XSeq<SyncWave> X{lds + w * REG};
    double2 v[V];
#pragma unroll
    for (int s = 0; s < V; ++s) {
        const int e = lane + s * 64;
        const double2 Xk = X.buf[XSeq<SyncWave>::idx(e)];
        const double2 Xm = cconj(X.buf[XSeq<SyncWave>::idx((n - e) & (n - 1))]);
        if (e == 0) {
            v[s] = make_double2(0.5 * (Xk.x + Xk.y), 0.5 * (Xk.x - Xk.y));
        } else {
            const double2 E = cscale(cadd(Xk, Xm), 0.5);
            const double2 O = cmulc(cscale(csub(Xk, Xm), 0.5), tw_M[e]);
            v[s] = make_double2(E.x - O.y, E.y + O.x);
        }
        if ((s & 3) == 3) __builtin_amdgcn_sched_barrier(0);
    }
    SyncWave::sync();
    stages_v<V, LOG2N, 0, true>(v, lane, tw_n1, X);
    const size_t colbase = ((size_t)b * N + j) * n;
    double2 *__restrict__ out = reinterpret_cast<double2 *>(x) + colbase;
    if constexpr (PM == 8) {
        double2 *__restrict__ yp = reinterpret_cast<double2 *>(post.ystep) + colbase;
        double2 yv[V];
#pragma unroll
        for (int s = 0; s < V; ++s) yv[s] = yp[lane + s * 64];
#pragma unroll
        for (int s = 0; s < V; ++s) {
            const double2 xv = cscale(v[s], scale);
            yp[lane + s * 64] = step_nocontract(yv[s], post.alpha, xv);
        }
    } else if constexpr ((PM & ~128) == 16) {
        if (post.marm.ctrl && blockIdx.x == 0 && threadIdx.x == 0) {
            ProxCtrl c = post.marm.ctrl[b];
            c.k = 0;
            c.done = 0;
            c.cur = 0;
            c.maxiter = post.marm.maxiter;
            c.redo = 0;
            c.f_valid = 0;
            c.err = 0.0;
            c.lambda = post.marm.lambda[b];
            c.tol = post.marm.tol;
            c.tau = post.marm.tau;
            post.marm.ctrl[b] = c;
        }
        double2 *__restrict__ xp = reinterpret_cast<double2 *>(post.ystep) + colbase;
        const double2 *__restrict__ pp = reinterpret_cast<const double2 *>(post.mprox) + colbase;
        const double2 *__restrict__ zp = post.mZ ? reinterpret_cast<const double2 *>(post.mZ) + colbase : nullptr;
        const double s2 = post.msig2[b];
        const unsigned step = post.mrng.step_dev ? (unsigned)post.mrng.step_dev[0] : post.mrng.step;
        const size_t q0 = (size_t)j * n;
        constexpr bool MOM = (PM & 128) != 0;
        int mk = 0;
        double mrk = 1.0;
        if constexpr (MOM) {
            mk = mom_sample(post.mom);
            mrk = 1.0 / (double)(mk > 0 ? mk : 1);
        }
        constexpr int CH = 4;
#pragma unroll
        for (int c0 = 0; c0 < V; c0 += CH) {
            double2 xv[CH], pv[CH], zv[CH];
#pragma unroll
            for (int q = 0; q < CH; ++q) {
                const int e = lane + (c0 + q) * 64;
                xv[q] = xp[e];
                pv[q] = pp[e];
                if (zp) zv[q] = zp[e];
            }
#pragma unroll
            for (int q = 0; q < CH; ++q) {
                const int e = lane + (c0 + q) * 64;
                if (!zp) zv[q] = philox_normal_pair(q0 + e, step, post.mrng.chain0 + (unsigned)b, post.mrng.seed);
                const double2 gv = cscale(v[c0 + q], scale);
                double2 r;
                r.x = myula_nocontract(xv[q].x, pv[q].x, gv.x, 1.0, zv[q].x, post.mgam, post.mlamb, s2, post.msq2g);
                r.y = myula_nocontract(xv[q].y, pv[q].y, gv.y, 1.0, zv[q].y, post.mgam, post.mlamb, s2, post.msq2g);
                xp[e] = r;
                if constexpr (MOM)
                    if (mk > 0) moments_pair(post.mom, 2 * (colbase + e), r, mk, mrk);
            }
            __builtin_amdgcn_sched_barrier(0);
        }
    } else if constexpr (PM == 64) {
        const double2 *__restrict__ bp = reinterpret_cast<const double2 *>(post.bu_in) + colbase;
        double2 *__restrict__ gp = reinterpret_cast<double2 *>(post.g) + colbase;
        double2 bb[V];
#pragma unroll
        for (int s = 0; s < V; ++s) bb[s] = bp[lane + s * 64];
#pragma unroll
        for (int s = 0; s < V; ++s) {
            const double2 xv = cscale(v[s], scale);
            out[lane + s * 64] = xv;
            gp[lane + s * 64] = make_double2(xv.x - bb[s].x, xv.y - bb[s].y);
        }
    } else if constexpr (!POST) {
#pragma unroll
        for (int s = 0; s < V; ++s) out[lane + s * 64] = cscale(v[s], scale);
    } else {
        constexpr int M = 2 * n;
        const size_t ibase = (size_t)b * N * M;
        const size_t cb = ibase + (size_t)j * M;
        const size_t cl = ibase + (size_t)(j > 0 ? j - 1 : N - 1) * M;
        const double *__restrict__ up_ = post.u + cb + 2 * lane, *__restrict__ ulp = post.u + cl + 2 * lane;
        double *__restrict__ bup = post.bu + cb + 2 * lane, *__restrict__ gp = post.g + cb + 2 * lane;
        const double *__restrict__ bin = NOX ? post.bu_in + cb + 2 * lane : nullptr;
        const double *__restrict__ trp = HAS_TRU ? post.tru + cb + 2 * lane : nullptr;
        const double *__restrict__ xpp = HAS_XPREV ? post.xprev + cb + 2 * lane : nullptr;
        double acc[6] = {0.0, 0.0, 0.0, 0.0, 0.0, 0.0};
        constexpr int CH = 2, NCH = V / CH;
        double2 ub[2][CH], bb[2][CH], tb[2][CH], lb[2][CH], xb[2][CH];
        auto fetch = [&](int c, int slot) {
#pragma unroll
            for (int q = 0; q < CH; ++q) {
                const int off = (c * CH + q) * 128;
                ub[slot][q] = *reinterpret_cast<const double2 *>(up_ + off);
                bb[slot][q] = *reinterpret_cast<const double2 *>((NOX ? bin : (const double *)bup) + off);
                lb[slot][q] = *reinterpret_cast<const double2 *>(ulp + off);
                if constexpr (HAS_TRU) tb[slot][q] = nt_load2(trp + off);
                if constexpr (HAS_XPREV) xb[slot][q] = *reinterpret_cast<const double2 *>(xpp + off);
            }
        };
        __builtin_amdgcn_sched_barrier(0);
        double carry = post.u[cb + M - 1];
        fetch(0, 0);
#pragma unroll
        for (int c = 0; c < NCH; ++c) {
            if (c + 1 < NCH) fetch(c + 1, (c + 1) & 1);
            __builtin_amdgcn_sched_barrier(0);
#pragma unroll
            for (int q = 0; q < CH; ++q) {
                const int s = c * CH + q, off = s * 128;
                const double2 xv = cscale(v[s], scale);
                if constexpr (!NOX) nt_store2(reinterpret_cast<double *>(out + lane + s * 64), xv);
                const double2 uv = ub[c & 1][q], ul = lb[c & 1][q];
                double2 bv = bb[c & 1][q];
                bv.x = bv.x + (uv.x - xv.x);
                bv.y = bv.y + (uv.y - xv.y);
                *reinterpret_cast<double2 *>(bup + off) = bv;
                *reinterpret_cast<double2 *>(gp + off) = make_double2(xv.x - bv.x, xv.y - bv.y);
                if constexpr (HAS_TRU) {
                    const double2 tv = tb[c & 1][q];
                    const double e0 = xv.x - tv.x, e1 = xv.y - tv.y;
                    acc[0] += e0 * e0 + e1 * e1;
                }
                const double d0 = xv.x - uv.x, d1 = xv.y - uv.y;
                acc[1] += d0 * d0 + d1 * d1;
                acc[2] += xv.x * xv.x + xv.y * xv.y;
                acc[3] += uv.x * uv.x + uv.y * uv.y;
                if constexpr (HAS_XPREV) {
                    const double2 xo = xb[c & 1][q];
                    const double p0 = xv.x - xo.x, p1 = xv.y - xo.y;
                    acc[4] += p0 * p0 + p1 * p1;
                }
                double upv = __shfl_up(uv.y, 1, 64);
                if (lane == 0) upv = carry;
                carry = __shfl(uv.y, 63, 64);
                const double h0 = uv.x - ul.x, v0 = uv.x - upv, h1 = uv.y - ul.y, v1 = uv.y - uv.x;
                acc[5] += sqrt(h0 * h0 + v0 * v0) + sqrt(h1 * h1 + v1 * v1);
            }
            __builtin_amdgcn_sched_barrier(0);
        }
#pragma unroll
        for (int c = 0; c < 6; ++c) {
#pragma unroll
            for (int off = 32; off > 0; off >>= 1) acc[c] += __shfl_xor(acc[c], off, 64);
        }
        if (lane == 0) {
#pragma unroll
            for (int c = 0; c < 6; ++c) post.partials[((size_t)b * 6 + c) * N + j] = acc[c];
        }
    }
}

template <int LOG2N, int OP>
__global__ __launch_bounds__((1 << LOG2N) / 4, 1) void rows_pipe_kernel(RowsParams p) {
    constexpr int N = 1 << LOG2N, V = 8, T = N / V, RK = 2, NT = RK * T, NW = NT / 64;
    constexpr int REG = N;
    constexpr bool needH = (OP != OP_NONE);
    constexpr bool CS = (OP == OP_CSALSA);
    constexpr bool needY = (OP == OP_SALSA || OP == OP_RESID || OP == OP_GRADF || OP == OP_GRAD || CS);
    constexpr bool needD = (OP == OP_GRAD);
    constexpr bool needD1 = needD || CS, noAhead = needD || CS;
#ifndef SBTV_CS_LATE_Y
#define SBTV_CS_LATE_Y 1
#endif
    constexpr bool lateY = CS && (SBTV_CS_LATE_Y != 0) && LOG2N == 11;
    __shared__ __attribute__((aligned(16))) double2 lds[RK * REG];
    __shared__ __attribute__((aligned(16))) double2 twl_buf[LdsTw::elems(N)];
    const LdsTw twl{twl_buf};
    __shared__ double red[3 * NW];
    const int fold = p.fold;
    const int ntk = fold ? (int)gridDim.x / fold : (int)gridDim.x;
    int b = blockIdx.y;
    int kb;
    {
        const int bid = blockIdx.x, xx = bid & 7;
        int o = bid >> 3;
        if (fold) {
            b = o % fold;
            o /= fold;
        }
        const int q8 = ntk >> 3, r8 = ntk & 7;
        kb = (xx < r8 ? xx * (q8 + 1) : r8 * (q8 + 1) + (xx - r8) * q8) + o;
    }
    if (p.frozen && p.frozen[b]) return;
    const int q = (threadIdx.x >> 5) & 1, t = (threadIdx.x & 31) | ((threadIdx.x >> 6) << 5);
    const int n1 = p.n1;
    const int k0 = kb * RK + q, k1 = (n1 >> 1) + kb * RK + q;
    const size_t ibase = (size_t)b * n1 * N;
    const double2 *__restrict__ in = p.Sin + ibase;
    double2 *__restrict__ out = p.Sout ? p.Sout + ibase : nullptr;
    XSwz<SyncBlock> X{lds + q * REG};
    const size_t hbase = p.shared_spec ? 0 : (size_t)b * p.u_img;
    const double mu = p.mu ? p.mu[b] : 0.0;
    const double2 z = make_double2(0.0, 0.0);
    const int sb = p.u_tiled ? 1 : n1 + 1, sc = p.u_tiled ? TW : 1;
    auto uidx = [&](int kk, int l) -> size_t {
        return hbase + (size_t)(l >> TWS) * (TW * (n1 + 1)) + (size_t)((l & (TW - 1)) * sb + kk * sc);
    };
    for (int i = threadIdx.x; i < N; i += NT) twl_buf[LdsTw::idx(i)] = p.tw[i];
    __syncthreads();

    double2 v[V], sn[V], h[V], y[V], d1[needD1 ? V : 1], d2[needD ? V : 1];
    if constexpr (!needD1) d1[0] = z;
    const CsPar cp = CS ? CsPar{p.cs[0], p.cs[1], p.cs[2]} : CsPar{0.0, 0.0, 0.0};
    auto apply = [&](double2 V_, double2 H_, double2 Y_, double2 &E_, double2 D2_, double wgt, double (&acc_)[3]) -> double2 {
        if constexpr (CS) return spec_apply_cs(V_, H_, Y_, E_, mu, cp, wgt, acc_);
        else return spec_apply<OP>(V_, H_, Y_, E_, D2_, mu, wgt, acc_);
    };
    auto dd1 = [&](int s) -> double2 & { return d1[needD1 ? s : 0]; };
    auto dd2 = [&](int s) -> double2 { return needD ? d2[needD ? s : 0] : z; };
#pragma unroll
    for (int s = 0; s < V; ++s) v[s] = in[s_tiled(k0, t + s * T, n1)];
    if constexpr (needH) {
#pragma unroll
        for (int s = 0; s < V; ++s) {
            h[s] = p.H[uidx(k0, t + s * T)];
            if constexpr (needY && !lateY) y[s] = p.Y[uidx(k0, t + s * T)];
            if constexpr (needD) {
                d1[s] = p.D1[uidx(k0, t + s * T)];
                d2[s] = p.D2[uidx(k0, t + s * T)];
            }
            if constexpr (CS) d1[s] = p.E[uidx(k0, t + s * T)];
        }
    }
    if constexpr (!noAhead) {
#pragma unroll
        for (int s = 0; s < V; ++s) sn[s] = in[s_tiled(k1, t + s * T, n1)];
    }
    double acc[3] = {0.0, 0.0, 0.0};

    if (p.fwd) stages_v<V, LOG2N, 0, false>(v, t, twl, X);
    if constexpr (lateY) {
#pragma unroll
        for (int s = 0; s < V; ++s) y[s] = p.Y[uidx(k0, t + s * T)];
    }
    if constexpr (needH) {
        if (kb == 0) {
#pragma unroll
            for (int s = 0; s < V; ++s) X.buf[XSwz<SyncBlock>::idx(t + s * T)] = v[s];
            SyncBlock::sync();
#pragma unroll
            for (int s = 0; s < V; ++s) {
                const int l = t + s * T;
                if (q == 0) {
                    const size_t hn = uidx(n1, l);
                    const double2 P = v[s], Q = cconj(X.buf[XSwz<SyncBlock>::idx((N - l) & (N - 1))]);
                    const double2 A = cscale(cadd(P, Q), 0.5);
                    const double2 dB = csub(P, Q);
                    const double2 B = make_double2(0.5 * dB.y, -0.5 * dB.x);
                    double2 en = needD ? p.D1[hn] : (CS ? p.E[hn] : z);
                    const double2 A2 = apply(A, h[s], needY ? y[s] : z, dd1(s), dd2(s), 1.0, acc);
                    const double2 B2 = apply(B, p.H[hn], needY ? p.Y[hn] : z, en, needD ? p.D2[hn] : z, 1.0, acc);
                    if constexpr (CS) p.E[hn] = en;
                    v[s] = make_double2(A2.x - B2.y, A2.y + B2.x);
                } else {
                    v[s] = apply(v[s], h[s], needY ? y[s] : z, dd1(s), dd2(s), 2.0, acc);
                }
                if constexpr (CS) p.E[uidx(k0, t + s * T)] = d1[s];
            }
            SyncBlock::sync();
        } else {
#pragma unroll
            for (int s = 0; s < V; ++s) {
                v[s] = apply(v[s], h[s], needY ? y[s] : z, dd1(s), dd2(s), 2.0, acc);
                if constexpr (CS) p.E[uidx(k0, t + s * T)] = d1[s];
            }
        }
        asm volatile("" : "+v"(acc[0]), "+v"(acc[1]), "+v"(acc[2]));
#pragma unroll
        for (int s = 0; s < V; ++s) {
            h[s] = p.H[uidx(k1, t + s * T)];
            if constexpr (needY && !lateY) y[s] = p.Y[uidx(k1, t + s * T)];
            if constexpr (needD) {
                d1[s] = p.D1[uidx(k1, t + s * T)];
                d2[s] = p.D2[uidx(k1, t + s * T)];
            }
            if constexpr (CS) d1[s] = p.E[uidx(k1, t + s * T)];
        }
    }
    if (p.inv) stages_v<V, LOG2N, 0, true>(v, t, twl, X);
    int ts = t;
    asm volatile("" : "+v"(ts));
    if (out) {
#pragma unroll
        for (int s = 0; s < V; ++s) out[s_tiled(k0, ts + s * T, n1)] = v[s];
    }
#pragma unroll
    for (int s = 0; s < V; ++s) v[s] = noAhead ? in[s_tiled(k1, t + s * T, n1)] : sn[s];
    if (p.fwd) stages_v<V, LOG2N, 0, false>(v, t, twl, X);
    if constexpr (lateY) {
#pragma unroll
        for (int s = 0; s < V; ++s) y[s] = p.Y[uidx(k1, t + s * T)];
    }
    if constexpr (needH) {
#pragma unroll
        for (int s = 0; s < V; ++s) {
            v[s] = apply(v[s], h[s], needY ? y[s] : z, dd1(s), dd2(s), 2.0, acc);
            if constexpr (CS) p.E[uidx(k1, t + s * T)] = d1[s];
        }
        asm volatile("" : "+v"(acc[0]), "+v"(acc[1]), "+v"(acc[2]));
    }
    if (p.inv) stages_v<V, LOG2N, 0, true>(v, t, twl, X);
    asm volatile("" : "+v"(ts));
    if (out) {
#pragma unroll
        for (int s = 0; s < V; ++s) out[s_tiled(k1, ts + s * T, n1)] = v[s];
    }
    if constexpr (needY) {
        const int lane = threadIdx.x & 63, w = threadIdx.x >> 6;
#pragma unroll
        for (int c = 0; c < 3; ++c) {
#pragma unroll
            for (int off = 32; off > 0; off >>= 1) acc[c] += __shfl_xor(acc[c], off, 64);
        }
        if (lane == 0) {
#pragma unroll
            for (int c = 0; c < 3; ++c) red[c * NW + w] = acc[c];
        }
        __syncthreads();
        if (threadIdx.x < 3) {
            double a = 0.0;
            for (int ww = 0; ww < NW; ++ww) a += red[threadIdx.x * NW + ww];
            p.acc[((size_t)b * 3 + threadIdx.x) * ntk + kb] = a;
        }
    }
}

__global__ void s_relayout_kernel(const double2 *__restrict__ in, double2 *__restrict__ out, int n1, int N, int to_tiled) {
    const size_t per = (size_t)n1 * N;
    const double2 *ib = in + (size_t)blockIdx.y * per;
    double2 *ob = out + (size_t)blockIdx.y * per;
    for (size_t q = (size_t)blockIdx.x * blockDim.x + threadIdx.x; q < per; q += (size_t)gridDim.x * blockDim.x) {
        const int c = (int)(q & (TW - 1));
        const size_t rest = q >> TWS;
        const int k = (int)(rest % n1), lt = (int)(rest / n1);
        const size_t plain = (size_t)(lt * TW + c) * n1 + k;
        if (to_tiled) ob[q] = ib[plain];
        else ob[plain] = ib[q];
    }
}

__global__ void spec_unpack_tiled_kernel(const double2 *__restrict__ S, double2 *__restrict__ U, int n1, int N, int utiled) {
    const int b = blockIdx.z;
    const int l = blockIdx.x * blockDim.x + threadIdx.x;
    const int k = blockIdx.y;
    if (l >= N) return;
    const double2 *s = S + (size_t)b * n1 * N;
    double2 *u = U + (size_t)b * (n1 + 1) * N;
    double2 r;
    if (k == 0 || k == n1) {
        const double2 P = s[s_tiled(0, l, n1)];
        const double2 Q = cconj(s[s_tiled(0, (N - l) & (N - 1), n1)]);
        if (k == 0) {
            r = cscale(cadd(P, Q), 0.5);
        } else {
            const double2 d = csub(P, Q);
            r = make_double2(0.5 * d.y, -0.5 * d.x);
        }
    } else {
        r = s[s_tiled(k, l, n1)];
    }
    if (utiled) u[u_tiled(k, l, n1)] = r;
    else u[(size_t)l * (n1 + 1) + k] = r;
}
```

semi-blind-image-deblurring-problems-with-tv_amd/csrc/operator.hip:

```cpp
#include "sbtv_internal.h"

namespace sbtv {

int op_open(sbtv_ctx *ctx, const char *prefix, int M, int N, int batch, const char *y_name, BlurOp *op) {
    SBTV_TRY(fft_plan(ctx, M, N, batch, &op->fp));
    op->batch = batch;
    op->P = (size_t)M * N;
    const std::string p = std::string(prefix) + ".";
    SBTV_TRY(ws_get_t(ctx, (p + "S").c_str(), (size_t)batch * op->fp.s_img, &op->S));
    SBTV_TRY(ws_get_t(ctx, (p + "H").c_str(), (size_t)batch * op->fp.u_img, &op->Hs));
    op->Ys = nullptr;
    if (y_name) SBTV_TRY(ws_get_t(ctx, (p + y_name).c_str(), (size_t)batch * op->fp.u_img, &op->Ys));
    op->inv_scale = 1.0 / ((double)op->fp.n1 * N);
    op->parseval = 1.0 / ((double)M * N);
    return 0;
}

int op_spectrum(sbtv_ctx *ctx, const FftPlan &fp, const double *in, const double *add, double2 *S, double2 *U) {
    RowsArgs a{};
    a.dir_fwd = 1;
    a.op = OP_NONE;
    SBTV_TRY(fft_cols_fwd(ctx, fp, in, add, S));
    SBTV_TRY(fft_rows(ctx, fp, S, S, a));
    return spec_unpack(ctx, fp, S, U);
}

static int op_through(sbtv_ctx *ctx, const BlurOp &c, const double *in, const double *add, RowsArgs a, double *out) {
    a.dir_fwd = a.dir_inv = 1;
    a.H = c.Hs;
    SBTV_TRY(fft_cols_fwd(ctx, c.fp, in, add, c.S));
    SBTV_TRY(fft_rows(ctx, c.fp, c.S, c.S, a));
    return fft_cols_inv(ctx, c.fp, c.S, out, c.inv_scale);
}

int op_apply(sbtv_ctx *ctx, const BlurOp &c, int op, const double *in, double *out, const double *mu) {
    RowsArgs a{};
    a.op = op;
    a.mu = mu;
    return op_through(ctx, c, in, nullptr, a, out);
}

int op_solve(sbtv_ctx *ctx, const BlurOp &c, const double *in, const double *add, const double2 *Y, const double *mu,
             double *acc, double *out) {
    RowsArgs a{};
    a.op = OP_SALSA;
    a.Y = Y;
    a.mu = mu;
    a.acc = acc;
    return op_through(ctx, c, in, add, a, out);
}

int op_gradf(sbtv_ctx *ctx, const BlurOp &c, const double *x, double *acc, double *grad) {
    RowsArgs a{};
    a.op = OP_GRADF;
    a.Y = c.Ys;
    a.acc = acc;
    return op_through(ctx, c, x, nullptr, a, grad);
}

int op_resid(sbtv_ctx *ctx, const BlurOp &c, const double *x, double *acc, const int *frozen, double *tvp) {
    RowsArgs a{};
    a.dir_fwd = 1;
    a.op = OP_RESID;
    a.H = c.Hs;
    a.Y = c.Ys;
    a.acc = acc;
    a.frozen = frozen;
    SBTV_TRY(fft_cols_fwd_f(ctx, c.fp, x, nullptr, c.S, frozen, tvp));
    return fft_rows(ctx, c.fp, c.S, nullptr, a);
}

int op_init_x(sbtv_ctx *ctx, const BlurOp &c, int initialization, const double *yd, const double *xi, double *x) {
    const size_t bytes = sizeof(double) * c.P * c.batch;
    if (initialization == 0) {
        SBTV_HIP(ctx, hipMemsetAsync(x, 0, bytes, ctx->stream));
    } else if (initialization == 2) {
        SBTV_TRY(op_apply(ctx, c, OP_MUL_HC, yd, x));
    } else {
        SBTV_HIP(ctx, hipMemcpyAsync(x, xi, bytes, hipMemcpyDeviceToDevice, ctx->stream));
    }
    return 0;
}

int check_psf_fits(sbtv_ctx *ctx, int taille, int M, int N) {
    if (taille < 1 || taille > 15 || taille > M || taille > N) return fail(ctx, SBTV_ERR_PSF, "Mask does not fit inside array");
    return 0;
}

int check_even_pixels(sbtv_ctx *ctx, int M, int N) {
    if (((size_t)M * N) & 1)
        return fail(ctx, SBTV_ERR_SIZE, "this entry point needs an even number of pixels (its element-wise passes move two per lane)");
    return 0;
}

int check_common(sbtv_ctx *ctx, const char *who, const double *y, const double *taps, const sbtv_salsa_opts *opts,
                 const double *x_init, int M, int N, int batch, int taille, const char *x_init_name, bool tv,
                 bool maxiter_positive) {
    if (!y || !opts || batch < 1) return fail(ctx, SBTV_ERR_BADARG, std::string(who) + ": missing required argument");
    if (!taps) return fail(ctx, SBTV_ERR_MISSING_AT, "The function handle for transpose of A is missing");
    if (opts->stopcriterion < 1 || opts->stopcriterion > 3) return fail(ctx, SBTV_ERR_STOPCRITERION, "Unknown stopping criterion");
    if (opts->initialization != 0 && opts->initialization != 2 && opts->initialization != 33333)
        return fail(ctx, SBTV_ERR_INIT, "Unknown 'Initialization' option");
    if (opts->initialization == 33333 && !x_init)
        return fail(ctx, SBTV_ERR_INIT, std::string("Initialization = array but ") + x_init_name + " is NULL");
    if (tv && opts->TViters <= 0) return fail(ctx, SBTV_ERR_MAXITER, std::string(who) + ": TViters must be positive");
    if (maxiter_positive && opts->maxiter < 1) return fail(ctx, SBTV_ERR_MAXITER, std::string(who) + ": maxiter must be positive");
    return check_psf_fits(ctx, taille, M, N);
}

}
```

semi-blind-image-deblurring-problems-with-tv_amd/csrc/salsa.hip:

```cpp
#include <algorithm>
#include <chrono>
#include <cmath>

#include <time.h>

#include "sbtv_internal.h"

namespace sbtv {

__global__ void salsa_setup_kernel(const double *__restrict__ src, double *__restrict__ par, int npar, int *__restrict__ frozen,
                                   int batch) {
    for (int i = threadIdx.x; i < npar; i += blockDim.x) par[i] = src[i];
    for (int b = threadIdx.x; b < batch; b += blockDim.x) frozen[b] = 0;
}

__global__ __launch_bounds__(256) void salsa_recover_x_kernel(const double *__restrict__ g, const double *__restrict__ bu,
                                                               double *__restrict__ x, size_t P) {
#pragma clang fp contract(off)
    for (size_t q = (size_t)blockIdx.x * 256 + threadIdx.x; q < P / 2; q += (size_t)gridDim.x * 256) {
        const double2 a = *reinterpret_cast<const double2 *>(g + 2 * q), b = *reinterpret_cast<const double2 *>(bu + 2 * q);
        *reinterpret_cast<double2 *>(x + 2 * q) = make_double2(a.x + b.x, a.y + b.y);
    }
}

__global__ __launch_bounds__(256) void salsa_collect_kernel(Collect c, ProxCtrl *__restrict__ ctrl,
                                                             unsigned long long out_addr,
                                                             const int *__restrict__ frozen, int rearm,
                                                             unsigned long long tags_addr, double seq) {
    __shared__ double red[4];
    salsa_collect_block(c, ctrl, out_addr, frozen, rearm, tags_addr, seq, blockIdx.x, blockIdx.y, red);
}

}

using namespace sbtv;

extern "C" {

void sbtv_salsa_opts_default(sbtv_salsa_opts *o) {
    if (!o) return;
    o->stopcriterion = 1;
    o->maxiter = 10000;
    o->TViters = 5;
    o->initialization = 0;
    o->compute_mse = 0;
    o->speculate = 1;
    o->tolA = 0.001;
    o->chambolle_tol = 1e-3;
    o->chambolle_tau = 0.249;
}

}

namespace {

struct SalsaRun {
    sbtv_ctx *ctx; const double *yd; int M, N, batch; const double *taps; int taille; const double *tau, *mu;
    const sbtv_salsa_opts *opts; const double *td, *xi; double *x_out, *objective, *distance, *times, *mses;
    int *numA, *numAt, *n_outer; int flags; bool spec_wanted;

    BlurOp op{};
    ProxPlan pp;
    size_t P = 0, cnt = 0, npar = 0;
    int maxiter = 0, lag = 0, nrb = 0, npb = 0, nl_prox = 0;
    bool want_mse = false, crit2 = false, zero_start = false, direct_last_ok = false, direct_last = false, nox = false,
         spec_ok = false, use_graph = false;
    double *xbuf[2] = {nullptr, nullptr}, *u = nullptr, *gb[2] = {nullptr, nullptr}, *bub[2] = {nullptr, nullptr};
    double *par = nullptr, *taps_d = nullptr, *mu_d = nullptr, *thr_d = nullptr;
    double *acc = nullptr, *postp = nullptr, *o4 = nullptr;
    int *frozen_d = nullptr;
    SalsaScal *scal_h = nullptr, *scal_hd = nullptr, *init_h = nullptr, *init_hd = nullptr;
    double *psum_h = nullptr, *psum_hd = nullptr, *tags_h = nullptr, *tags_hd = nullptr, *init_tags_h = nullptr,
           *init_tags_hd = nullptr;
    int *frozen_h = nullptr;
    hipEvent_t ev_done[2], ev_p0[2], ev_p1[2];

    std::vector<int> h_numA, h_numAt, frozen, h_nouter;
    std::vector<double> obj_prev;
    bool init_read = false;
    int active = 0;
    double ms_prox = 0.0;
    long long prox_iters_run = 0, prox_iters_timed = 0;
    GraphExecs graphs;
    std::chrono::steady_clock::time_point t0;
    bool prox_timed[2] = {false, false}, slot_tagged[2] = {false, false}, slot_spec[2] = {false, false};
    struct PendingCollect {
        bool valid = false;
        int outer = 0;
        bool spec = false;
    } pend;

    int open() {
        SBTV_TRY(op_open(ctx, "salsa", M, N, batch, "Y", &op));
        SBTV_TRY(prox_plan(ctx, M, N, batch, &pp));
        P = op.P;
        cnt = P * batch;
        maxiter = opts->maxiter;
        want_mse = (td != nullptr);
        crit2 = (opts->stopcriterion == 2);
        zero_start = (opts->initialization == 0);
        lag = (opts->speculate & 1) ? 1 : 0;
        SBTV_TRY(ws_get_t(ctx, "salsa.x0", cnt, &xbuf[0]));
        SBTV_TRY(ws_get_t(ctx, "salsa.x1", cnt, &xbuf[1]));
        direct_last_ok = x_out && (flags & SBTV_DEVICE_PTRS) && !graph_wanted(cnt) && !overlaps(yd, x_out, cnt) &&
                         !overlaps(td, x_out, cnt) && !overlaps(xi, x_out, cnt);
        SBTV_TRY(ws_get_t(ctx, "salsa.u", cnt, &u));
        SBTV_TRY(ws_get_t(ctx, "salsa.bu", cnt, &bub[0]));
        SBTV_TRY(ws_get_t(ctx, "salsa.g", cnt, &gb[0]));
        static const bool env_nox = [] {
            const char *e = getenv("SBTV_SALSA_NOX");
            return !(e && e[0] == '0');
        }();
        nox = env_nox && fft_cols_inv_step_ok(op.fp) && !crit2 && !graph_wanted(cnt) && x_out != nullptr;
        gb[1] = gb[0];
        bub[1] = bub[0];
        if (nox) {
            SBTV_TRY(ws_get_t(ctx, "salsa.bu1", cnt, &bub[1]));
            SBTV_TRY(ws_get_t(ctx, "salsa.g1", cnt, &gb[1]));
        }
        direct_last = direct_last_ok && !nox;
        const size_t nt = (size_t)batch * taille * taille;
        npar = nt + 2 * (size_t)batch;
        SBTV_TRY(ws_get_t(ctx, "salsa.par", npar, &par));
        taps_d = par;
        mu_d = par + nt;
        thr_d = mu_d + batch;
        SBTV_TRY(ws_get_t(ctx, "salsa.frozen", (size_t)batch, &frozen_d));
        nrb = fft_rows_blocks(op.fp);
        npb = fft_cols_blocks(op.fp);
        SBTV_TRY(ws_get_t(ctx, "salsa.acc", (size_t)batch * 3 * nrb, &acc));
        SBTV_TRY(ws_get_t(ctx, "salsa.post", (size_t)batch * 6 * npb, &postp));
        SalsaScal *scal_d = nullptr;
        SBTV_TRY(ws_get_t(ctx, "salsa.scal", 2 * (size_t)batch, &scal_d));
        SBTV_TRY(ws_get_t(ctx, "salsa.o4", (size_t)batch * 4, &o4));

        PinnedLayout lay;
        const auto f_scal = lay.add<SalsaScal>(2 * (size_t)batch);
        const auto f_init = lay.add<SalsaScal>((size_t)batch);
        const auto f_psum = lay.add<double>(2 * (size_t)batch * FSTRIDE);
        const auto f_tags = lay.add<double>(2 * (size_t)batch * SALSA_TAGS);
        const auto f_itag = lay.add<double>((size_t)batch * SALSA_TAGS);
        const auto f_par = lay.add<double>(npar);
        const auto f_frozen = lay.add<int>((size_t)batch);
        void *ph = nullptr, *pd = nullptr;
        SBTV_TRY(pinned_get(ctx, lay.bytes(), &ph, &pd));
        scal_h = f_scal.at(ph), scal_hd = f_scal.at(pd);
        init_h = f_init.at(ph), init_hd = f_init.at(pd);
        psum_h = f_psum.at(ph), psum_hd = f_psum.at(pd);
        tags_h = f_tags.at(ph), tags_hd = f_tags.at(pd);
        init_tags_h = f_itag.at(ph), init_tags_hd = f_itag.at(pd);
        frozen_h = f_frozen.at(ph);
        for (int b = 0; b < batch; ++b) frozen_h[b] = 0;
        for (size_t i = 0; i < f_tags.count; ++i) tags_h[i] = 0.0;
        for (size_t i = 0; i < f_itag.count; ++i) init_tags_h[i] = 0.0;
        double *par_stage = f_par.at(ph);
        for (size_t q = 0; q < nt; ++q) par_stage[q] = taps[q];
        for (int b = 0; b < batch; ++b) {
            par_stage[nt + b] = mu[b];
            par_stage[nt + batch + b] = tau[b] / mu[b];
        }
        hipLaunchKernelGGL(salsa_setup_kernel, dim3(1), dim3(256), 0, ctx->stream, (const double *)f_par.at(pd), par, (int)npar,
                           frozen_d, batch);
        SBTV_HIP(ctx, hipGetLastError());
        return 0;
    }

    int spectra() {
        const long long dims[6] = {M, N, batch, taille, op.fp.u_tiled, (long long)op.fp.u_img};
        const size_t nt = (size_t)batch * taille * taille;
        const bool same = ctx->salsa_h_ptr == (const void *)op.Hs && std::equal(dims, dims + 6, ctx->salsa_h_dims) &&
                          ctx->salsa_h_taps.size() == nt && std::equal(taps, taps + nt, ctx->salsa_h_taps.begin());
        if (!same) {
            ctx->salsa_h_ptr = nullptr;
            SBTV_TRY(psf_spectrum(ctx, op.fp, taps_d, taille, op.Hs));
            ctx->salsa_h_taps.assign(taps, taps + nt);
            std::copy(dims, dims + 6, ctx->salsa_h_dims);
            ctx->salsa_h_ptr = (const void *)op.Hs;
        }
        SBTV_TRY(op_spectrum(ctx, op.fp, yd, nullptr, op.S, op.Ys));
        h_numA.assign(batch, 0);
        h_numAt.assign(batch, 1);
        ctx->calls += 2LL * batch;
        return 0;
    }

    int start() {
        double *x = xbuf[0], *bu = bub[0], *g = gb[0];
        if (zero_start) ctx->calls += batch;
        else SBTV_TRY(op_init_x(ctx, op, opts->initialization, yd, xi, x));
        if (!zero_start) {
            SBTV_HIP(ctx, hipMemcpyAsync(u, x, sizeof(double) * cnt, hipMemcpyDeviceToDevice, ctx->stream));
            SBTV_HIP(ctx, hipMemcpyAsync(g, x, sizeof(double) * cnt, hipMemcpyDeviceToDevice, ctx->stream));
            SBTV_HIP(ctx, hipMemsetAsync(bu, 0, sizeof(double) * cnt, ctx->stream));
        }
        SBTV_TRY(prox_reset(ctx, pp, thr_d, 1.0, opts->TViters, opts->chambolle_tol, opts->chambolle_tau, false, nullptr));
        obj_prev.assign(batch, 0.0);
        Collect c{};
        if (zero_start) {
            double *accz = nullptr, *postz = nullptr;
            int nz = 0;
            SBTV_TRY(salsa_zero_start(ctx, yd, want_mse ? td : nullptr, x, u, bu, P, batch, (double)M * (double)N, &accz, &postz,
                                      &nz));
            c = Collect{accz, nz, nullptr, 0, postz, nz, nullptr, 0, 0, 0ull, nullptr};
        } else {
            double *tvp = nullptr;
            int ntv = 0;
            RowsArgs a{};
            a.dir_fwd = 1;
            a.op = OP_RESID;
            a.H = op.Hs;
            a.Y = op.Ys;
            a.acc = acc;
            SBTV_TRY(fft_cols_fwd(ctx, op.fp, x, nullptr, op.S));
            SBTV_TRY(tvnorm_partials(ctx, u, M, N, batch, &tvp, &ntv));
            SBTV_TRY(fft_rows(ctx, op.fp, op.S, nullptr, a));
            if (want_mse) SBTV_TRY(pair_sums(ctx, x, td, P, batch, o4));
            c = Collect{acc, nrb, tvp, ntv, nullptr, 0, nullptr, 0, 0, 0ull, want_mse ? o4 : nullptr};
        }
        hipLaunchKernelGGL(salsa_collect_kernel, dim3(7, batch), dim3(256), 0, ctx->stream, c, (ProxCtrl *)nullptr,
                           (unsigned long long)(uintptr_t)init_hd, (const int *)nullptr, 0,
                           (unsigned long long)(uintptr_t)init_tags_hd, 1.0);
        SBTV_HIP(ctx, hipGetLastError());
        ctx->calls += batch;
        return 0;
    }

    int read_initial() {
        if (init_read) return 0;
        init_read = true;
        volatile const double *tg = init_tags_h;
        for (unsigned spin = 0;; ++spin) {
            bool ready = true;
            for (int b = 0; b < batch && ready; ++b)
                for (int i = 0; i < 8 && ready; ++i) ready = (tg[(size_t)b * SALSA_TAGS + i] == 1.0);
            if (ready) break;
            if (spin > 2000) {
                SBTV_HIP(ctx, hipStreamSynchronize(ctx->stream));
                break;
            }
            struct timespec ts = {0, 5000};
            nanosleep(&ts, nullptr);
        }
        __atomic_thread_fence(__ATOMIC_ACQUIRE);
        for (int b = 0; b < batch; ++b) {
            h_numA[b] += 1;
            const double f0 = 0.5 * (init_h[b].resid2 * op.parseval) + tau[b] * init_h[b].tv_u;
            obj_prev[b] = f0;
            if (objective) objective[(size_t)b * (maxiter + 1)] = f0;
            if (times) times[(size_t)b * (maxiter + 1)] = 0.0;
            if (mses && want_mse) mses[(size_t)b * (maxiter + 1)] = init_h[b].mse_num / (double)P;
        }
        return 0;
    }

    Collect make_collect(int outer, bool spec) const {
        const int slot = outer & 1;
        return Collect{acc, nrb, nullptr, 0, postp, npb, spec ? pp.partials + (size_t)slot * pp.part_stride : nullptr, pp.fnblk,
                       opts->TViters, (unsigned long long)(uintptr_t)(psum_hd + (size_t)slot * batch * FSTRIDE), nullptr};
    }
    int launch_collect(int outer, bool spec, bool tagged) {
        const int slot = outer & 1;
        const Collect c = make_collect(outer, spec);
        hipLaunchKernelGGL(salsa_collect_kernel, dim3(spec ? 7 + opts->TViters : 7, batch), dim3(256), 0, ctx->stream, c, pp.ctrl,
                           (unsigned long long)(uintptr_t)(scal_hd + (size_t)slot * batch), (const int *)frozen_d, 1,
                           tagged ? (unsigned long long)(uintptr_t)(tags_hd + (size_t)slot * batch * SALSA_TAGS) : 0ull, (double)outer);
        SBTV_HIP(ctx, hipGetLastError());
        return 0;
    }
    int flush_pending() {
        if (!pend.valid) return 0;
        pend.valid = false;
        return launch_collect(pend.outer, pend.spec, true);
    }

    int enqueue_body(int outer, bool eager) {
        static const bool piggyback = [] {
            const char *e = getenv("SBTV_COLLECT_RIDE");
            return !(e && e[0] == '0');
        }();
        const int slot = outer & 1;
        const bool tagged = eager;
        const bool spec = spec_ok && outer >= 2;
        const bool timed = eager && ((outer & 31) == 4 || outer == 12);
        slot_tagged[slot] = tagged;
        slot_spec[slot] = spec;
        double *xn = (direct_last && outer == maxiter) ? x_out : xbuf[slot];
        const double *xprev = xbuf[slot ^ 1];
        SideJob side{};
        if (pend.valid && spec) {
            const int ps = pend.outer & 1;
            side.c = make_collect(pend.outer, pend.spec);
            side.out_addr = (unsigned long long)(uintptr_t)(scal_hd + (size_t)ps * batch);
            side.tags_addr = (unsigned long long)(uintptr_t)(tags_hd + (size_t)ps * batch * SALSA_TAGS);
            side.frozen = frozen_d;
            side.seq = (double)pend.outer;
            side.nblocks = 7 + (pend.spec ? opts->TViters : 0);
            pend.valid = false;
        } else {
            SBTV_TRY(flush_pending());
        }
        if (timed) SBTV_HIP(ctx, hipEventRecord(ev_p0[slot], ctx->stream));
        ProxPlan pps = pp;
        pps.partials = pp.partials + (size_t)slot * pp.part_stride;
        if (!(zero_start && outer == 1))
            SBTV_TRY(prox_iterate(ctx, pps, gb[(outer - 1) & 1], opts->TViters, u, outer == (zero_start ? 2 : 1), spec,
                                  spec ? ((outer - 2) * nl_prox) & 1 : 0, side.nblocks ? &side : nullptr));
        if (timed) SBTV_HIP(ctx, hipEventRecord(ev_p1[slot], ctx->stream));
        prox_timed[slot] = timed;
        RowsArgs a{};
        a.dir_fwd = 1;
        a.dir_inv = 1;
        a.op = OP_SALSA;
        a.H = op.Hs;
        a.Y = op.Ys;
        a.mu = mu_d;
        a.acc = acc;
        a.frozen = frozen_d;
        SBTV_TRY(fft_cols_fwd_f(ctx, op.fp, u, bub[(outer - 1) & 1], op.S, frozen_d));
        SBTV_TRY(fft_rows(ctx, op.fp, op.S, op.S, a));
        ColsPost cp;
        cp.u = u;
        cp.bu = bub[outer & 1];
        cp.g = gb[outer & 1];
        if (nox) {
            cp.bu_in = bub[(outer - 1) & 1];
            cp.skip_x = 1;
        }
        cp.tru = td;
        cp.xprev = crit2 ? xprev : nullptr;
        cp.partials = postp;
        SBTV_TRY(fft_cols_inv_post(ctx, op.fp, op.S, xn, op.inv_scale, frozen_d, cp));
        if (spec && eager && lag == 1 && outer < maxiter && piggyback) {
            pend.valid = true;
            pend.outer = outer;
            pend.spec = spec;
            return 0;
        }
        return launch_collect(outer, spec, tagged);
    }
    int enqueue(int outer) {
        const int slot = outer & 1;
        hipGraphExec_t(&gexec)[2] = graphs.g;
        if (use_graph && outer >= 3) {
            if (!gexec[slot]) {
                if (graph_begin(ctx) != 0 || graph_end(ctx, enqueue_body(outer, false), &gexec[slot]) != 0) {
                    use_graph = false;
                    gexec[slot] = nullptr;
                }
            }
            if (gexec[slot]) {
                SBTV_HIP(ctx, hipGraphLaunch(gexec[slot], ctx->stream));
                SBTV_HIP(ctx, hipEventRecord(ev_done[slot], ctx->stream));
                return 0;
            }
        }
        return enqueue_body(outer, true);
    }

    int process(int outer) {
        const int slot = outer & 1;
        SBTV_TRY(read_initial());
        if (pend.valid && pend.outer == outer) SBTV_TRY(flush_pending());
        if (slot_tagged[slot])
            SBTV_TRY(wait_tags(ctx, tags_h + (size_t)slot * batch * SALSA_TAGS, batch, SALSA_TAGS, 8,
                               slot_spec[slot] ? opts->TViters : 0, (double)outer));
        else SBTV_TRY(wait_event(ctx, ev_done[slot]));
        if (prox_timed[slot]) {
            float ms = 0.f;
            SBTV_HIP(ctx, hipEventSynchronize(ev_p1[slot]));
            SBTV_HIP(ctx, hipEventElapsedTime(&ms, ev_p0[slot], ev_p1[slot]));
            ms_prox += ms;
            for (int b = 0; b < batch; ++b)
                if (!frozen[b]) prox_iters_timed += slot_spec[slot] ? (long long)opts->TViters : (long long)scal_h[(size_t)slot * batch + b].pad;
            prox_timed[slot] = false;
        }
        if (slot_spec[slot])
            SBTV_TRY(spec_stop_rule(ctx, pp, psum_h + (size_t)slot * batch * FSTRIDE, opts->TViters, opts->chambolle_tol,
                                    frozen.data()));
        const double tnow = std::chrono::duration<double>(std::chrono::steady_clock::now() - t0).count();
        bool changed = false;
        for (int b = 0; b < batch; ++b) {
            if (frozen[b]) continue;
            const SalsaScal &s = scal_h[(size_t)slot * batch + b];
            h_numA[b] += 1;
            h_nouter[b] = outer;
            double prox_k = s.pad;
            if (zero_start && outer == 1) prox_k = 1.0;
            if (slot_spec[slot]) prox_k = (double)opts->TViters;
            prox_iters_run += (long long)prox_k;
            ctx->calls += 2;
            const double f = 0.5 * (s.resid2 * op.parseval) + tau[b] * s.tv_u;
            if (objective) objective[(size_t)b * (maxiter + 1) + outer] = f;
            if (mses && want_mse) mses[(size_t)b * (maxiter + 1) + outer] = s.mse_num / (double)P;
            if (distance) distance[(size_t)b * maxiter + (outer - 1)] = sqrt(s.dist_num) / sqrt(s.x2 + s.u2);
            if (times) times[(size_t)b * (maxiter + 1) + outer] = tnow;
            const bool stop = salsa_stop(opts->stopcriterion, outer, f, obj_prev[b], s.dx2, s.x2, opts->tolA);
            obj_prev[b] = f;
            if (stop) {
                frozen[b] = 1;
                frozen_h[b] = 1;
                --active;
                changed = true;
            }
        }
        if (changed && active > 0) SBTV_TRY(upload_frozen(ctx, frozen_h, frozen_d, batch, pp.ctrl));
        return 0;
    }

    int result() {
        if (!x_out) return 0;
        for (int b = 0; b < batch; ++b) {
            double *out = x_out + (size_t)b * P;
            if (!nox) {
                if (direct_last && h_nouter[b] == maxiter) continue;
                const double *src = xbuf[h_nouter[b] & 1] + (size_t)b * P;
                if (flags & SBTV_DEVICE_PTRS)
                    SBTV_HIP(ctx, hipMemcpyAsync(out, src, sizeof(double) * P, hipMemcpyDeviceToDevice, ctx->stream));
                else
                    SBTV_TRY(stage_out_copy(ctx, out, src, P, flags));
                continue;
            }
            const int par = h_nouter[b] & 1;
            const bool dev_direct = direct_last_ok;
            double *dst = dev_direct ? out : xbuf[0] + (size_t)b * P;
            const int nblk = (int)std::min<size_t>((P / 2 + 255) / 256, 2048);
            if (h_nouter[b] == 0) {
                SBTV_HIP(ctx, hipMemcpyAsync(dst, xbuf[0] + (size_t)b * P, sizeof(double) * P, hipMemcpyDeviceToDevice, ctx->stream));
            } else {
                hipLaunchKernelGGL(salsa_recover_x_kernel, dim3(nblk), dim3(256), 0, ctx->stream,
                                   (const double *)(gb[par] + (size_t)b * P), (const double *)(bub[par] + (size_t)b * P), dst, P);
                SBTV_HIP(ctx, hipGetLastError());
            }
            if (!dev_direct && (flags & SBTV_DEVICE_PTRS))
                SBTV_HIP(ctx, hipMemcpyAsync(out, dst, sizeof(double) * P, hipMemcpyDeviceToDevice, ctx->stream));
            else if (!dev_direct)
                SBTV_TRY(stage_out_copy(ctx, out, dst, P, flags));
        }
        return 0;
    }

    int finish() {
        SBTV_TRY(loop_timing(ctx, prox_iters_timed > 0 ? ms_prox * ((double)prox_iters_run / (double)prox_iters_timed) : 0.0,
                             prox_iters_run, batch, P));
        for (int b = 0; b < batch; ++b) {
            if (numA) numA[b] = h_numA[b];
            if (numAt) numAt[b] = h_numAt[b];
            if (n_outer) n_outer[b] = h_nouter[b];
        }
        return 0;
    }

    int run() {
        SBTV_TRY(open());
        SBTV_TRY(spectra());
        SBTV_TRY(start());
        frozen.assign(batch, 0);
        h_nouter.assign(batch, 0);
        active = batch;
        for (auto &e : ctx->loop_ev)
            if (!e) SBTV_HIP(ctx, hipEventCreate(&e));
        for (int s = 0; s < 2; ++s) {
            ev_done[s] = ctx->loop_ev[s];
            ev_p0[s] = ctx->loop_ev[2 + s];
            ev_p1[s] = ctx->loop_ev[4 + s];
        }
        t0 = std::chrono::steady_clock::now();
        spec_ok = spec_wanted && !graph_wanted(cnt) && prox_spec_ok(pp, gb[0], u, opts->TViters);
        nl_prox = prox_launches(pp, opts->TViters);
        use_graph = graph_wanted(cnt);
        int done = 0;
        SBTV_TRY(pipelined_loop(ctx, &done, maxiter, lag, true, [&](int k) { return enqueue(k); }, [&](int k) { return process(k); },
                                [&] { return active > 0; }));
        SBTV_TRY(read_initial());
        SBTV_HIP(ctx, hipEventRecord(ctx->ev[1], ctx->stream));
        SBTV_TRY(result());
        SBTV_HIP(ctx, hipStreamSynchronize(ctx->stream));
        return finish();
    }
};

}

extern "C" int sbtv_SALSA_v2(sbtv_ctx *ctx, const double *y, int M, int N, int batch, const double *taps, int taille,
                             const double *tau, const double *mu, const sbtv_salsa_opts *opts, const double *true_x,
                             const double *x_init, double *x_out, double *objective, double *distance, double *times,
                             double *mses, int *numA, int *numAt, int *n_outer, int flags) {
    if (!ctx) return SBTV_ERR_BADARG;
    if (!tau || !mu) return fail(ctx, SBTV_ERR_BADARG, "SALSA_v2: missing required argument");
    SBTV_TRY(check_common(ctx, "SALSA_v2", y, taps, opts, x_init, M, N, batch, taille, "x_init", true, false));
    for (int b = 0; b < batch; ++b)
        if (!(mu[b] > 0.0)) return fail(ctx, SBTV_ERR_MISSING_LS, "(A^T A + mu I)^(-1) must be specified: mu must be > 0");
    SBTV_HIP(ctx, hipSetDevice(ctx->device));
    if (sbtv_group *lg = lanes_group(ctx, batch, false)) {
        LaneCall lc(ctx, lg);
        return lc.done(salsa_sharded(lg, y, M, N, batch, taps, taille, tau, mu, opts, true_x, x_init, x_out, objective,
                                     distance, times, mses, numA, numAt, n_outer, flags), batch);
    }
    SBTV_HIP(ctx, hipEventRecord(ctx->ev[0], ctx->stream));
    const size_t cnt = (size_t)M * N * batch;
    const double *yd = nullptr, *td = nullptr, *xi = nullptr;
    SBTV_TRY(stage_in(ctx, "salsa.y", y, cnt, flags, &yd));
    SBTV_TRY(stage_in(ctx, "salsa.true", true_x, cnt, flags, &td));
    SBTV_TRY(stage_in(ctx, "salsa.xinit", x_init, cnt, flags, &xi));
    return canary_epilogue(ctx, solve_with_exact_repeat(ctx, !(opts->speculate & 2), [&](bool spec) {
        SalsaRun r{ctx, yd, M, N, batch, taps, taille, tau, mu, opts, td, xi, x_out, objective, distance, times, mses,
                   numA, numAt, n_outer, flags, spec};
        return r.run();
    }));
}
```

semi-blind-image-deblurring-problems-with-tv_amd/csrc/sbtv_internal.h:

```cpp
#pragma once
#include <hip/hip_runtime.h>

#include <chrono>
#include <map>
#include <string>
#include <vector>

#include "../../include/sbtv.h"
#include "pinned_layout.h"

namespace sbtv {

constexpr int kWave = 64;

struct ProxCtrl {
    int k;
    int done;
    int cur;
    int maxiter;
    int redo;
    int f_valid;
    double err;
    double lambda;
    double tol;
// ... 302 lines not shown
                   int taille, const double *tau, const double *mu1, const double *mu2, const sbtv_salsa_opts *opts,
                   const double *true_x, const double *x_init, double *x_out, double *objective, double *distance,
                   double *times, double *mses, int *numA, int *numAt, int *n_outer, int flags);

int wait_event(sbtv_ctx *ctx, hipEvent_t ev);
int wait_stream(sbtv_ctx *ctx);
int wait_tags(sbtv_ctx *ctx, const double *tags, int batch, int stride, int nscal, int nstep, double seq);

bool graph_wanted(size_t total_px);
int graph_begin(sbtv_ctx *ctx);
int graph_end(sbtv_ctx *ctx, int body_rc, hipGraphExec_t *exec);
struct GraphExecs {
    hipGraphExec_t g[2] = {nullptr, nullptr};
    ~GraphExecs() {
        for (auto e : g)
            if (e) (void)hipGraphExecDestroy(e);
    }
};

int loop_timing(sbtv_ctx *ctx, double prox_ms, long long prox_iters, int batch, size_t P);
void host_stats_begin(sbtv_ctx *ctx);
void host_stats_end(sbtv_ctx *ctx);

template <class Enqueue, class Process, class Active>
int pipelined_loop(sbtv_ctx *ctx, int *done, int maxiter, int lag, bool stats, Enqueue &&enqueue, Process &&process,
                   Active &&active) {
    if (stats) host_stats_begin(ctx);
    int rc = 0, enq = *done;
    while (rc == 0 && active() && *done < maxiter) {
        while (rc == 0 && enq < maxiter && enq - *done <= lag) {
            const auto te = std::chrono::steady_clock::now();
            rc = enqueue(++enq);
            const double d = std::chrono::duration<double>(std::chrono::steady_clock::now() - te).count();
            if (stats) {
                ctx->hstat.enqueue_s += d;
                if (d > ctx->hstat.enqueue_max_s) ctx->hstat.enqueue_max_s = d;
            }
        }
        if (rc == 0) rc = process(++*done);
    }
    if (rc != 0) {
        (void)hipStreamSynchronize(ctx->stream);
        return rc;
    }
    if (stats) host_stats_end(ctx);
    return 0;
}

struct ProxPlan {
    int M, N, batch;
    int tiles_i, tiles_j, nblk;
    int ftiles_i, ftiles_j, fnblk;
    int cj, nw, minw, rpl;
    ProxCtrl *ctrl;
    double *pbuf;
    int pairs;
    std::string tag;
    double *partials;
    size_t part_stride;
    unsigned *counters;
    const int *order;
    int esub_off;
};
int prox_plan(sbtv_ctx *ctx, int M, int N, int batch, ProxPlan *plan, const char *tag = "prox");
int prox_reset(sbtv_ctx *ctx, const ProxPlan &pl, const double *lambda_dev, double lambda_scale,
               int maxiter, double tol, double tau, bool keep_cur, const int *frozen);
int prox_zero_duals(sbtv_ctx *ctx, const ProxPlan &pl);
int prox_set_duals(sbtv_ctx *ctx, const ProxPlan &pl, const double *px, const double *py);
int prox_get_duals(sbtv_ctx *ctx, const ProxPlan &pl, double *px, double *py);
constexpr int FSMAX = 10;
constexpr double SPEC_TOL_GUARD = 1.0 + 1e-12;
constexpr double ESUB_MARGIN = 32.0;
constexpr int FSTRIDE = 32;
constexpr int SALSA_TAGS = 8 + FSTRIDE;
struct Collect {
    const double *acc;
    int nrb;
    const double *tvp;
    int ntv;
    const double *post;
    int npb;
    const double *ppart;
    int pnblk, psteps;
    unsigned long long psum_addr;
    const double *mse0;
};
struct SideJob {
    Collect c;
    unsigned long long out_addr, tags_addr;
    const int *frozen;
    double seq;
    int nblocks;
};
#ifdef __HIPCC__
#include "collect.inc"
#endif

int prox_iterate(sbtv_ctx *ctx, const ProxPlan &pl, const double *g, int maxiter, double *f_out = nullptr,
                 bool cold = false, int spec = 0, int spec_parity = 0, const SideJob *side = nullptr);
int prox_reserve_pairs(sbtv_ctx *ctx, ProxPlan *pl, int pairs);
int prox_launches(const ProxPlan &pl, int maxiter);
bool prox_spec_ok(const ProxPlan &pl, const double *g, const double *f_out, int maxiter);
constexpr double CHAMBOLLE_TOL = 1e-3, CHAMBOLLE_TAU = 0.249;

constexpr int SOLVE_RESTART_EXACT = 12345;
int spec_stop_rule(sbtv_ctx *ctx, ProxPlan &pp, const double *stepsums, int K, double tol, const int *frozen = nullptr);
template <class Body>
int solve_with_exact_repeat(sbtv_ctx *ctx, bool spec, Body &&body) {
    const long long calls0 = ctx->calls;
    const int rc = body(spec);
    if (rc != SOLVE_RESTART_EXACT) return rc;
    ctx->calls = calls0;
    ctx->solve_stats[0] += 1;
    return body(false);
}
int upload_frozen(sbtv_ctx *ctx, const int *frozen_h, int *frozen_d, int batch, ProxCtrl *park_ctrl);
int prox_finish(sbtv_ctx *ctx, const ProxPlan &pl, const double *g, double *f);
int tvnorm_dev(sbtv_ctx *ctx, const double *x, int M, int N, int batch, double *out_dev);
int tvnorm_partials(sbtv_ctx *ctx, const double *x, int M, int N, int batch, double **partials, int *nblk);

enum SpecOp {
    OP_NONE = 0,
    OP_MUL_H = 1,
    OP_MUL_HC = 2,
    OP_INVLS = 3,
    OP_SALSA = 4,
    OP_RESID = 5,
    OP_GRAD = 6,
    OP_ATA = 7,
    OP_GRADF = 8,
    OP_CSALSA = 9,
};
struct FftPlan {
    int M, N, batch;
    int n1;
    int wave;
    int u_tiled;
    size_t u_img;
    size_t s_img;
    int generic;
    const double2 *tw_n1;
    const double2 *tw_M;
    const double2 *tw_N;
};
int fft_plan(sbtv_ctx *ctx, int M, int N, int batch, FftPlan *plan);
int fft_cols_fwd(sbtv_ctx *ctx, const FftPlan &pl, const double *x, const double *add, double2 *S);
int fft_cols_inv(sbtv_ctx *ctx, const FftPlan &pl, const double2 *S, double *x, double scale);
struct ColsPost {
    const double *u = nullptr;
    double *bu = nullptr;
    double *g = nullptr;
    const double *bu_in = nullptr;
    int skip_x = 0;
    const double *tru = nullptr;
    const double *xprev = nullptr;
    double *partials = nullptr;
    double *ystep = nullptr;
    double alpha = 0.0;
    const double *mprox = nullptr, *msig2 = nullptr, *mZ = nullptr;
    double mgam = 0.0, mlamb = 0.0, msq2g = 0.0;
    RngArgs mrng = {0ull, 0u, 0u, nullptr};
    ProxArm marm = {nullptr, nullptr, 0, 0.0, 0.0, nullptr};
    MomArgs mom = {nullptr, nullptr, 0, nullptr, 1, 1};
};
int fft_cols_inv_myula(sbtv_ctx *ctx, const FftPlan &pl, const double2 *S, double scale, double *X, const double *prox,
                       const double *Z, const double *sigma2_dev, double gam, double lamb, const RngArgs *rng,
                       const ProxArm *arm, const MomArgs *mom = nullptr);
int fft_cols_blocks(const FftPlan &pl);
bool fft_cols_inv_step_ok(const FftPlan &pl);
int fft_cols_inv_step(sbtv_ctx *ctx, const FftPlan &pl, const double2 *S, double *y, double scale, double alpha,
                      const int *frozen);
int fft_cols_inv_sub(sbtv_ctx *ctx, const FftPlan &pl, const double2 *S, double *x, double scale, const double *b, double *g);
int fft_cols_inv_post(sbtv_ctx *ctx, const FftPlan &pl, const double2 *S, double *x, double scale, const int *frozen,
                      const ColsPost &post);
struct RowsArgs {
    int dir_fwd;
    int dir_inv;
    int op;
    const double2 *H;
    const double2 *Y;
    const double2 *D1, *D2;
    double2 *E;
    const double *cs;
    const double *mu;
    double *acc;
    const int *frozen;
    int shared_spec;
};
int fft_rows(sbtv_ctx *ctx, const FftPlan &pl, const double2 *Sin, double2 *Sout, const RowsArgs &a);
int fft_rows_blocks(const FftPlan &pl);
bool fft_rows_csalsa_ok(const FftPlan &pl);
int spec_unpack(sbtv_ctx *ctx, const FftPlan &pl, const double2 *S, double2 *U);
int psf_spectrum(sbtv_ctx *ctx, const FftPlan &pl, const double *taps_dev, int taille, double2 *U);
int psf_spectrum_sets(sbtv_ctx *ctx, const FftPlan &pl, const double *const *taps_dev, int taille, double2 *const *U, int nsets);

int reduce_partials(sbtv_ctx *ctx, const double *partials, int nvec, int n, double *out);
struct RedJobs {
    const double *src[4] = {nullptr, nullptr, nullptr, nullptr};
    double *dst[4] = {nullptr, nullptr, nullptr, nullptr};
    int nvec[4] = {0, 0, 0, 0};
    int n[4] = {0, 0, 0, 0};
    int dropped = 0;
    void add(const double *s, int nv, int nn, double *d) {
        for (int q = 0; q < 4; ++q)
            if (nvec[q] == 0) {
                src[q] = s;
                dst[q] = d;
                nvec[q] = nv;
                n[q] = nn;
                return;
            }
        ++dropped;
    }
};
int reduce_jobs(sbtv_ctx *ctx, const RedJobs &jb);
int ew_blocks(size_t P);
int pair_sums(sbtv_ctx *ctx, const double *a, const double *c, size_t P, int batch, double *out4_dev);
int salsa_zero_start(sbtv_ctx *ctx, const double *y, const double *tru, double *x, double *u, double *bu, size_t P, int batch,
                     double scale, double **accp, double **postp, int *nblk);
int axpy(sbtv_ctx *ctx, double *y, const double *gr, double a, size_t Ptot, const ProxArm *arm = nullptr, int batch = 0);
int fista_momentum(sbtv_ctx *ctx, const double *x, const double *xold, double *y, const double *tru, double coef,
                   double *partials, size_t P, int batch, const int *frozen);
int myula_step(sbtv_ctx *ctx, double *X, const double *prox, const double *grad, const double *Z,
               const double *sigma2_dev, double gam, double lamb, size_t P, int batch, const RngArgs *rng = nullptr,
               const ProxArm *arm = nullptr, const MomArgs *mom = nullptr);
int myula_plain_step(sbtv_ctx *ctx, double *X, const double *prox, const double *grad, const double *Z,
                     const double *sigma2_dev, double gam, double lamb, size_t P, int batch, const RngArgs *rng,
                     const ProxArm *arm, const MomArgs *mom = nullptr);
int fft_cols_fwd_f(sbtv_ctx *ctx, const FftPlan &pl, const double *x, const double *add, double2 *S, const int *frozen,
                   double *tvp = nullptr);
bool fft_cols_tv_ok(const FftPlan &pl);
int fft_cols_inv_f(sbtv_ctx *ctx, const FftPlan &pl, const double2 *S, double *x, double scale, const int *frozen);

struct BlurOp {
    FftPlan fp;
    int batch;
    size_t P;
    double2 *S, *Hs, *Ys;
    double inv_scale, parseval;
};
int op_open(sbtv_ctx *ctx, const char *prefix, int M, int N, int batch, const char *y_name, BlurOp *op);
int op_spectrum(sbtv_ctx *ctx, const FftPlan &fp, const double *in, const double *add, double2 *S, double2 *U);
int op_apply(sbtv_ctx *ctx, const BlurOp &c, int op, const double *in, double *out, const double *mu = nullptr);
int op_solve(sbtv_ctx *ctx, const BlurOp &c, const double *in, const double *add, const double2 *Y, const double *mu,
             double *acc, double *out);
int op_resid(sbtv_ctx *ctx, const BlurOp &c, const double *x, double *acc, const int *frozen = nullptr, double *tvp = nullptr);
int op_gradf(sbtv_ctx *ctx, const BlurOp &c, const double *x, double *acc, double *grad);
int op_init_x(sbtv_ctx *ctx, const BlurOp &c, int initialization, const double *yd, const double *xi, double *x);

int check_psf_fits(sbtv_ctx *ctx, int taille, int M, int N);
int check_even_pixels(sbtv_ctx *ctx, int M, int N);
int check_common(sbtv_ctx *ctx, const char *who, const double *y, const double *taps, const sbtv_salsa_opts *opts,
                 const double *x_init, int M, int N, int batch, int taille, const char *x_init_name = "x_init", bool tv = true,
                 bool maxiter_positive = true);
inline bool salsa_stop(int stopcriterion, int outer, double f, double obj_prev, double num, double den, double tolA) {
    if (outer <= 1) return false;
    double crit;
    if (stopcriterion == 1)
        crit = fabs(f - obj_prev) / obj_prev;
    else if (stopcriterion == 2)
        crit = fabs(sqrt(num) / sqrt(den));
    else
        crit = f;
    return crit < tolA;
}

struct WavPlan {
    int M, N, K, J;
    double f0[8], f1[8];
    int bands() const { return 3 * J + 1; }
};
int wav_plan(sbtv_ctx *ctx, int M, int N, const double *h, int hlen, int levels, bool orthonormal, WavPlan *pl);
int wav_analysis(sbtv_ctx *ctx, const WavPlan &pl, const double *x, double *z, int batch);
int wav_synthesis(sbtv_ctx *ctx, const WavPlan &pl, const double *z, double *x, int batch);
int wav_synthesis(sbtv_ctx *ctx, const WavPlan &pl, const double *z, double *x, int batch, const MomArgs *mom);
__device__ __forceinline__ double wav_soft(double x, double T) { return copysign(fmax(fabs(x) - T, 0.0), x); }
__device__ __forceinline__ double wav_myula_nocontract(double x, double g, double z, double T, double gam, double lamb,
                                                       double s2, double sq2g) {
#pragma clang fp contract(off)
    return ((x + gam * (wav_soft(x, T) - x) / lamb) - gam * (g / s2)) + sq2g * z;
}
constexpr int WAV_EWB = 256;
constexpr int WAV_EW_MAXBLK = 2048;
inline int wav_ew_blocks(size_t dimX) {
    const size_t nb = (dimX / 2 + WAV_EWB - 1) / WAV_EWB;
    return nb > (size_t)WAV_EW_MAXBLK ? WAV_EW_MAXBLK : (nb < 1 ? 1 : (int)nb);
}
__device__ __forceinline__ double wav_wave_sum(double v) {
#pragma unroll
    for (int off = 32; off > 0; off >>= 1) v += __shfl_xor(v, off, 64);
    return v;
}
__device__ __forceinline__ double wav_block_sum(double v, double *red) {
    v = wav_wave_sum(v);
    __syncthreads();
    if ((threadIdx.x & 63) == 0) red[threadIdx.x >> 6] = v;
    __syncthreads();
    return (red[0] + red[1]) + (red[2] + red[3]);
}
struct WavThetaStep {
    double eta, th;
    double sum_eta, n_eta;
    double tol, mean;
};
__device__ __forceinline__ WavThetaStep wav_theta_step(double eta, double th_cur, double g, double delta, double dimX,
                                                       double min_eta, double max_eta, bool burn, double sum_eta,
                                                       double n_eta) {
#pragma clang fp contract(off)
    WavThetaStep t;
    const double etaii = eta + delta * (dimX / th_cur - g) * exp(eta);
    t.eta = fmin(fmax(etaii, min_eta), max_eta);
    t.th = exp(t.eta);
    const double nan = __builtin_nan("");
    const double m0 = n_eta > 0.0 ? exp(sum_eta / n_eta) : nan;
    t.sum_eta = burn ? sum_eta + t.eta : sum_eta;
    t.n_eta = burn ? n_eta + 1.0 : n_eta;
    t.mean = t.n_eta > 0.0 ? exp(t.sum_eta / t.n_eta) : nan;
    t.tol = fabs(t.mean - m0) / m0;
    return t;
}

struct WavChain {
    WavPlan wp;
    BlurOp op;
    int batch, nblk, nrb;
    size_t P, cnt, dimX, ccnt;
    const double *yd, *x0d;
    const double *noise;
    double *X, *G, *img, *Z;
};
int wav_chain_buffers(sbtv_ctx *ctx, const char *prefix, const WavPlan &wp, int batch, const double *y, const double *xw0,
                      const double *noise, double *xw_last, int flags, WavChain *c);
int wav_chain_start(sbtv_ctx *ctx, const WavChain &c);
int wav_chain_spectrum(sbtv_ctx *ctx, const WavChain &c, const MomArgs *mom = nullptr);
int wav_chain_rows(sbtv_ctx *ctx, const WavChain &c, int op, double *acc, const double2 *D1 = nullptr,
                   const double2 *D2 = nullptr);
int wav_abs_sum(sbtv_ctx *ctx, const WavChain &c, double *part);
struct WavStepPar {
    const double *theta, *sigma2;
    int stride;
// ... 23 lines not shown
```

Measured before the change: 4636 SALSA outer-iterations/s.

## Skip zero-state clears and first-iteration loads in SALSA start and last iteration

The first SALSA outer iteration now uses specialised kernel instances: the row pass treats a known-zero spectrum as input, and the column post pass treats bu as zero, so the zero-fill of x/u/bu, two device copies and the first forward column FFT can be skipped. The prox reset is folded into the setup kernel. On the last iteration the no-x path rebuilds x straight into the output buffer, which removes a separate recover/copy. This adds many template instances and validity checks, and depends on first-iteration buffers never being read before they are written.

After: 4632 SALSA outer-iterations/s. Within noise of the previous version (-0.1%).

```diff
diff --git a/semi-blind-image-deblurring-problems-with-tv_amd/csrc/ctx.hip b/semi-blind-image-deblurring-problems-with-tv_amd/csrc/ctx.hip
--- a/semi-blind-image-deblurring-problems-with-tv_amd/csrc/ctx.hip
+++ b/semi-blind-image-deblurring-problems-with-tv_amd/csrc/ctx.hip
@@ -524,7 +524,8 @@
         "SBTV_CANARY", "SBTV_COLLECT_RIDE", "SBTV_EXACT", "SBTV_FFT_WAVE", "SBTV_FISTA_FUSED_STEP", "SBTV_FISTA_LAG",
         "SBTV_FUSED_VARIANT", "SBTV_GRAPH", "SBTV_INLINE_CTRL", "SBTV_PROX_SPEC", "SBTV_SAPG_DEFER",
         "SBTV_SAPG_FUSED_MYULA", "SBTV_SAPG_HOST", "SBTV_SINGLE_STEP", "SBTV_SPIN", "SBTV_TAG_SPIN_US", "SBTV_TILE_ORDER", "SBTV_SALSA_NOX", "SBTV_CSALSA_SPECTRAL",
-        "SBTV_CORAL_BATCH", "SBTV_ROWS_FOLD", "SBTV_ERR_SUBSET", "SBTV_LANES", "SBTV_LANE_COUNT", "SBTV_STAGE_THREADS", "SBTV_TEST_FAIL_SAPG", "SBTV_FUSED_STAGGER"};
+        "SBTV_CORAL_BATCH", "SBTV_ROWS_FOLD", "SBTV_ERR_SUBSET", "SBTV_LANES", "SBTV_LANE_COUNT", "SBTV_STAGE_THREADS", "SBTV_TEST_FAIL_SAPG", "SBTV_FUSED_STAGGER",
+        "SBTV_SALSA_DIRECT_LAST", "SBTV_SALSA_ZERO_FAST"};
     if (!buf || cap == 0) return SBTV_ERR_BADARG;
     std::string s;
     int nset = 0;
diff --git a/semi-blind-image-deblurring-problems-with-tv_amd/csrc/elementwise.hip b/semi-blind-image-deblurring-problems-with-tv_amd/csrc/elementwise.hip
--- a/semi-blind-image-deblurring-problems-with-tv_amd/csrc/elementwise.hip
+++ b/semi-blind-image-deblurring-problems-with-tv_amd/csrc/elementwise.hip
@@ -34,6 +34,7 @@
     return (int)nb;
 }
 
+template <bool CLEAR>
 __global__ __launch_bounds__(EWB) void salsa_zero_start_kernel(const double *__restrict__ y, const double *__restrict__ tru,
                                                                 double *__restrict__ x, double *__restrict__ u,
                                                                 double *__restrict__ bu, double *__restrict__ accp,
@@ -47,9 +48,11 @@
         const double tv = tru ? tru[base + q] : 0.0;
         acc[0] += yv * yv;
         acc[1] += tv * tv;
-        x[base + q] = 0.0;
-        u[base + q] = 0.0;
-        bu[base + q] = 0.0;
+        if constexpr (CLEAR) {
+            x[base + q] = 0.0;
+            u[base + q] = 0.0;
+            bu[base + q] = 0.0;
+        }
     }
     ew_block_sum<2>(acc, red);
     if (threadIdx.x == 0) {
@@ -319,8 +322,14 @@
     const int G = ew_blocks(2 * P);
     SBTV_TRY(ws_get_t(ctx, "ew.zero.acc", (size_t)batch * 3 * G, accp));
     SBTV_TRY(ws_get_t(ctx, "ew.zero.post", (size_t)batch * 6 * G, postp));
-    hipLaunchKernelGGL(salsa_zero_start_kernel, dim3(G, batch), dim3(EWB), 0, ctx->stream, y, tru, x, u, bu, *accp, *postp, P,
-                       scale);
+    if ((x == nullptr) != (u == nullptr) || (x == nullptr) != (bu == nullptr))
+        return fail(ctx, SBTV_ERR_BADARG, "salsa_zero_start: x, u and bu are cleared together or not at all");
+    if (x)
+        hipLaunchKernelGGL(salsa_zero_start_kernel<true>, dim3(G, batch), dim3(EWB), 0, ctx->stream, y, tru, x, u, bu, *accp,
+                           *postp, P, scale);
+    else
+        hipLaunchKernelGGL(salsa_zero_start_kernel<false>, dim3(G, batch), dim3(EWB), 0, ctx->stream, y, tru, x, u, bu, *accp,
+                           *postp, P, scale);
     SBTV_HIP(ctx, hipGetLastError());
     *nblk = G;
     return 0;
diff --git a/semi-blind-image-deblurring-problems-with-tv_amd/csrc/fft.hip b/semi-blind-image-deblurring-problems-with-tv_amd/csrc/fft.hip
--- a/semi-blind-image-deblurring-problems-with-tv_amd/csrc/fft.hip
+++ b/semi-blind-image-deblurring-problems-with-tv_amd/csrc/fft.hip
@@ -440,6 +440,8 @@
     int fold;
     size_t u_img;
     int u_tiled;
+    int s_zero;
+    double2 *U;
 };
 
 template <int OP>
@@ -1007,15 +1009,24 @@
 int fft_cols_blocks(const FftPlan &pl) { return (pl.wave || pl.generic) ? pl.N : pl.N / cols_nseq(pl); }
 int fft_cols_inv_post(sbtv_ctx *ctx, const FftPlan &pl, const double2 *S, double *x, double scale, const int *frozen,
                       const ColsPost &post) {
-    if ((!pl.wave && (post.bu_in || post.skip_x)) || (post.bu_in && !post.skip_x))
-        return fail(ctx, SBTV_ERR_BADARG, "fft_cols_inv_post: bu_in + skip_x go together and need the wave-granular column pass");
+    if (!pl.wave && (post.bu_in || post.skip_x || post.recover_x || post.zero_in || post.zero_bu))
+        return fail(ctx, SBTV_ERR_BADARG,
+                    "fft_cols_inv_post: bu_in, skip_x, recover_x, zero_in and zero_bu need the wave-granular column pass");
+    if (post.zero_bu && (post.zero_in || post.bu_in))
+        return fail(ctx, SBTV_ERR_BADARG, "fft_cols_inv_post: zero_bu reads no bu (not with bu_in or zero_in)");
     if (pl.generic) return any_cols_inv(ctx, pl, S, x, scale, frozen, &post);
     if (pl.wave) {
         const PassDims cd = cols_dims(pl);
         const dim3 grid(cd.wgs, pl.batch), block(cd.threads);
-        if (post.skip_x && (!post.bu_in || post.bu_in == post.bu || post.xprev))
+        if (post.skip_x && ((!post.zero_in && !post.zero_bu && (!post.bu_in || post.bu_in == post.bu)) || post.xprev))
             return fail(ctx, SBTV_ERR_BADARG, "fft_cols_inv_post: skip_x needs a separate bu_in and no xprev");
-        const int pm = 1 + (post.tru ? 2 : 0) + (post.xprev ? 4 : 0) + (post.skip_x ? 32 : 0);
+        const bool bin_x = post.recover_x != 0;
+        if (bin_x && (post.skip_x || post.xprev || (!post.zero_in && !post.zero_bu && (!post.bu_in || post.bu_in == post.bu))))
+            return fail(ctx, SBTV_ERR_BADARG, "fft_cols_inv_post: recover_x needs a separate bu_in, no skip_x and no xprev");
+        if (post.bu_in && !post.skip_x && !bin_x)
+            return fail(ctx, SBTV_ERR_BADARG, "fft_cols_inv_post: bu_in goes with skip_x or recover_x");
+        const int pm = 1 + (post.tru ? 2 : 0) + (post.xprev ? 4 : 0) + (post.skip_x ? 32 : 0) + (post.zero_in ? 256 : 0) +
+                       (bin_x ? 512 : 0) + (post.zero_bu ? 1024 : 0);
 #define SBTV_POST_CASE(PM_)                                                                                          \
     case PM_:                                                                                                        \
         if (pl.n1 == 1024)                                                                                           \
@@ -1032,6 +1043,25 @@
             SBTV_POST_CASE(7)
             SBTV_POST_CASE(33)
             SBTV_POST_CASE(35)
+            SBTV_POST_CASE(1 + 256)
+            SBTV_POST_CASE(3 + 256)
+            SBTV_POST_CASE(5 + 256)
+            SBTV_POST_CASE(7 + 256)
+            SBTV_POST_CASE(33 + 256)
+            SBTV_POST_CASE(35 + 256)
+            SBTV_POST_CASE(1 + 512)
+            SBTV_POST_CASE(3 + 512)
+            SBTV_POST_CASE(1 + 256 + 512)
+            SBTV_POST_CASE(3 + 256 + 512)
+            SBTV_POST_CASE(1 + 1024 + 512)
+            SBTV_POST_CASE(3 + 1024 + 512)
+            SBTV_POST_CASE(1 + 1024)
+            SBTV_POST_CASE(3 + 1024)
+            SBTV_POST_CASE(5 + 1024)
+            SBTV_POST_CASE(7 + 1024)
+            SBTV_POST_CASE(33 + 1024)
+            SBTV_POST_CASE(35 + 1024)
+            default: return fail(ctx, SBTV_ERR_BADARG, "fft_cols_inv_post: no such instance of the bookkeeping pass");
         }
 #undef SBTV_POST_CASE
         SBTV_HIP(ctx, hipGetLastError());
@@ -1083,6 +1113,14 @@
     const dim3 grid(fold ? rd.wgs * pl.batch : rd.wgs, fold ? 1 : pl.batch), block(rd.threads);
 #define SBTV_ROWS_OP(OP_)                                                                                     \
     case OP_: hipLaunchKernelGGL((rows_pipe_kernel<L, OP_>), grid, block, 0, ctx->stream, p); break;
+    if (p.s_zero) {
+        hipLaunchKernelGGL((rows_pipe_kernel<L, OP_SALSA + ROWS_ZS>), grid, block, 0, ctx->stream, p);
+        return;
+    }
+    if (p.U) {
+        hipLaunchKernelGGL((rows_pipe_kernel<L, OP_NONE + ROWS_UNP>), grid, block, 0, ctx->stream, p);
+        return;
+    }
     switch (p.op) {
         SBTV_ROWS_OP(OP_NONE)
         SBTV_ROWS_OP(OP_MUL_H)
@@ -1143,7 +1181,13 @@
     p.fold = 0;
     p.u_img = pl.u_img;
     p.u_tiled = pl.u_tiled;
+    p.s_zero = a.s_zero;
+    p.U = a.U;
+    if (a.U && (!pl.wave || pl.generic || !pl.u_tiled || a.op != OP_NONE || !a.dir_fwd || a.dir_inv || a.shared_spec))
+        return fail(ctx, SBTV_ERR_BADARG, "row pass: the unpacking instance is the forward OP_NONE of the pipelined row kernel");
     SBTV_TRY(fft_rows_check(ctx, pl, a.op));
+    if (a.s_zero && (!pl.wave || pl.generic || a.op != OP_SALSA || !a.dir_inv))
+        return fail(ctx, SBTV_ERR_BADARG, "row pass: the zero-input instance is OP_SALSA of the pipelined row kernel");
     if (pl.generic) return any_rows(ctx, pl, p, Sout);
     const int L = ilog2(pl.N);
     if (L > 12) return fail(ctx, SBTV_ERR_SIZE, "row FFT: N must be <= 4096");
diff --git a/semi-blind-image-deblurring-problems-with-tv_amd/csrc/fft_wave.inc b/semi-blind-image-deblurring-problems-with-tv_amd/csrc/fft_wave.inc
--- a/semi-blind-image-deblurring-problems-with-tv_amd/csrc/fft_wave.inc
+++ b/semi-blind-image-deblurring-problems-with-tv_amd/csrc/fft_wave.inc
@@ -243,6 +243,12 @@
     constexpr int n = 1 << LOG2N;
     constexpr bool POST = (PM & 1) != 0, HAS_TRU = (PM & 2) != 0, HAS_XPREV = (PM & 4) != 0;
     constexpr bool NOX = (PM & 32) != 0;
+    constexpr bool ZIN = (PM & 256) != 0;
+    constexpr bool BZ = (PM & 1024) != 0;
+    constexpr bool RECX = (PM & 512) != 0;
+    constexpr bool BIN = (NOX || RECX) && !ZIN && !BZ;
+    static_assert(!(NOX && RECX), "an x that is not stored has no stored form");
+    static_assert(!(BZ && (BIN || ZIN)), "a zero bu is not read from anywhere");
     static_assert(n == 64 * V, "one wave per column");
     constexpr int REG = xseq_elems(n);
     __shared__ __attribute__((aligned(16))) double2 lds[TW * REG];
@@ -368,24 +374,57 @@
         const size_t cl = ibase + (size_t)(j > 0 ? j - 1 : N - 1) * M;
         const double *__restrict__ up_ = post.u + cb + 2 * lane, *__restrict__ ulp = post.u + cl + 2 * lane;
         double *__restrict__ bup = post.bu + cb + 2 * lane, *__restrict__ gp = post.g + cb + 2 * lane;
-        const double *__restrict__ bin = NOX ? post.bu_in + cb + 2 * lane : nullptr;
+        const double *__restrict__ bin = BIN ? post.bu_in + cb + 2 * lane : nullptr;
         const double *__restrict__ trp = HAS_TRU ? post.tru + cb + 2 * lane : nullptr;
         const double *__restrict__ xpp = HAS_XPREV ? post.xprev + cb + 2 * lane : nullptr;
         double acc[6] = {0.0, 0.0, 0.0, 0.0, 0.0, 0.0};
         constexpr int CH = 2, NCH = V / CH;
         double2 ub[2][CH], bb[2][CH], tb[2][CH], lb[2][CH], xb[2][CH];
+        double zb = 0.0;
+        if constexpr (BZ) asm volatile("" : "+v"(zb));
         auto fetch = [&](int c, int slot) {
 #pragma unroll
             for (int q = 0; q < CH; ++q) {
                 const int off = (c * CH + q) * 128;
                 ub[slot][q] = *reinterpret_cast<const double2 *>(up_ + off);
-                bb[slot][q] = *reinterpret_cast<const double2 *>((NOX ? bin : (const double *)bup) + off);
+                if constexpr (BZ) bb[slot][q] = make_double2(zb, zb);
+                else bb[slot][q] = *reinterpret_cast<const double2 *>((BIN ? bin : (const double *)bup) + off);
                 lb[slot][q] = *reinterpret_cast<const double2 *>(ulp + off);
                 if constexpr (HAS_TRU) tb[slot][q] = nt_load2(trp + off);
                 if constexpr (HAS_XPREV) xb[slot][q] = *reinterpret_cast<const double2 *>(xpp + off);
             }
         };
         __builtin_amdgcn_sched_barrier(0);
+        if constexpr (ZIN) {
+            double zo = 0.0;
+            asm volatile("" : "+v"(zo));
+#pragma unroll
+            for (int s = 0; s < V; ++s) {
+                const int off = s * 128;
+                const double2 xv = cscale(v[s], scale);
+                if constexpr (!NOX && !RECX) nt_store2(reinterpret_cast<double *>(out + lane + s * 64), xv);
+                const double2 uv = make_double2(zo, zo);
+                double2 bv = make_double2(zo, zo);
+                bv.x = bv.x + (uv.x - xv.x);
+                bv.y = bv.y + (uv.y - xv.y);
+                *reinterpret_cast<double2 *>(bup + off) = bv;
+                const double2 gv = make_double2(xv.x - bv.x, xv.y - bv.y);
+                *reinterpret_cast<double2 *>(gp + off) = gv;
+                if constexpr (RECX) nt_store2(reinterpret_cast<double *>(out + lane + s * 64), make_double2(gv.x + bv.x, gv.y + bv.y));
+                if constexpr (HAS_TRU) {
+                    const double2 tv = nt_load2(trp + off);
+                    const double e0 = xv.x - tv.x, e1 = xv.y - tv.y;
+                    acc[0] += e0 * e0 + e1 * e1;
+                }
+                const double d0 = xv.x - uv.x, d1 = xv.y - uv.y;
+                acc[1] += d0 * d0 + d1 * d1;
+                acc[2] += xv.x * xv.x + xv.y * xv.y;
+                if constexpr (HAS_XPREV) {
+                    const double p0 = xv.x - zo, p1 = xv.y - zo;
+                    acc[4] += p0 * p0 + p1 * p1;
+                }
+            }
+        } else {
         double carry = post.u[cb + M - 1];
         fetch(0, 0);
 #pragma unroll
@@ -396,13 +435,15 @@
             for (int q = 0; q < CH; ++q) {
                 const int s = c * CH + q, off = s * 128;
                 const double2 xv = cscale(v[s], scale);
-                if constexpr (!NOX) nt_store2(reinterpret_cast<double *>(out + lane + s * 64), xv);
+                if constexpr (!NOX && !RECX) nt_store2(reinterpret_cast<double *>(out + lane + s * 64), xv);
                 const double2 uv = ub[c & 1][q], ul = lb[c & 1][q];
                 double2 bv = bb[c & 1][q];
                 bv.x = bv.x + (uv.x - xv.x);
                 bv.y = bv.y + (uv.y - xv.y);
                 *reinterpret_cast<double2 *>(bup + off) = bv;
-                *reinterpret_cast<double2 *>(gp + off) = make_double2(xv.x - bv.x, xv.y - bv.y);
+                const double2 gv = make_double2(xv.x - bv.x, xv.y - bv.y);
+                *reinterpret_cast<double2 *>(gp + off) = gv;
+                if constexpr (RECX) nt_store2(reinterpret_cast<double *>(out + lane + s * 64), make_double2(gv.x + bv.x, gv.y + bv.y));
                 if constexpr (HAS_TRU) {
                     const double2 tv = tb[c & 1][q];
                     const double e0 = xv.x - tv.x, e1 = xv.y - tv.y;
@@ -425,6 +466,7 @@
             }
             __builtin_amdgcn_sched_barrier(0);
         }
+        }
 #pragma unroll
         for (int c = 0; c < 6; ++c) {
 #pragma unroll
@@ -437,8 +479,14 @@
     }
 }
 
-template <int LOG2N, int OP>
+constexpr int ROWS_ZS = 32, ROWS_UNP = 64;
+template <int LOG2N, int OPX>
 __global__ __launch_bounds__((1 << LOG2N) / 4, 1) void rows_pipe_kernel(RowsParams p) {
+    constexpr int OP = OPX & 31;
+    constexpr bool ZS = (OPX & ROWS_ZS) != 0, UNP = (OPX & ROWS_UNP) != 0;
+    static_assert((OPX & ~(31 | ROWS_ZS | ROWS_UNP)) == 0, "SpecOp + mode bits");
+    static_assert(!ZS || OP == OP_SALSA, "the zero-input row pass exists for OP_SALSA");
+    static_assert(!UNP || OP == OP_NONE, "the unpacking row pass applies no operator");
     constexpr int N = 1 << LOG2N, V = 8, T = N / V, RK = 2, NT = RK * T, NW = NT / 64;
     constexpr int REG = N;
     constexpr bool needH = (OP != OP_NONE);
@@ -479,6 +527,9 @@
     const size_t hbase = p.shared_spec ? 0 : (size_t)b * p.u_img;
     const double mu = p.mu ? p.mu[b] : 0.0;
     const double2 z = make_double2(0.0, 0.0);
+    double zo = 0.0;
+    if constexpr (ZS) asm volatile("" : "+v"(zo));
+    const double2 zs = make_double2(zo, zo);
     const int sb = p.u_tiled ? 1 : n1 + 1, sc = p.u_tiled ? TW : 1;
     auto uidx = [&](int kk, int l) -> size_t {
         return hbase + (size_t)(l >> TWS) * (TW * (n1 + 1)) + (size_t)((l & (TW - 1)) * sb + kk * sc);
@@ -496,7 +547,7 @@
     auto dd1 = [&](int s) -> double2 & { return d1[needD1 ? s : 0]; };
     auto dd2 = [&](int s) -> double2 { return needD ? d2[needD ? s : 0] : z; };
 #pragma unroll
-    for (int s = 0; s < V; ++s) v[s] = in[s_tiled(k0, t + s * T, n1)];
+    for (int s = 0; s < V; ++s) v[s] = ZS ? zs : in[s_tiled(k0, t + s * T, n1)];
     if constexpr (needH) {
 #pragma unroll
         for (int s = 0; s < V; ++s) {
@@ -509,13 +560,13 @@
             if constexpr (CS) d1[s] = p.E[uidx(k0, t + s * T)];
         }
     }
-    if constexpr (!noAhead) {
+    if constexpr (!noAhead && !ZS) {
 #pragma unroll
         for (int s = 0; s < V; ++s) sn[s] = in[s_tiled(k1, t + s * T, n1)];
     }
     double acc[3] = {0.0, 0.0, 0.0};
 
-    if (p.fwd) stages_v<V, LOG2N, 0, false>(v, t, twl, X);
+    if (!ZS && p.fwd) stages_v<V, LOG2N, 0, false>(v, t, twl, X);
     if constexpr (lateY) {
 #pragma unroll
         for (int s = 0; s < V; ++s) y[s] = p.Y[uidx(k0, t + s * T)];
@@ -567,13 +618,35 @@
     if (p.inv) stages_v<V, LOG2N, 0, true>(v, t, twl, X);
     int ts = t;
     asm volatile("" : "+v"(ts));
-    if (out) {
+    if constexpr (UNP) {
+        if (kb == 0) {
+#pragma unroll
+            for (int s = 0; s < V; ++s) X.buf[XSwz<SyncBlock>::idx(t + s * T)] = v[s];
+            SyncBlock::sync();
+#pragma unroll
+            for (int s = 0; s < V; ++s) {
+                const int l = t + s * T;
+                if (q == 0) {
+                    const double2 P = v[s], Q = cconj(X.buf[XSwz<SyncBlock>::idx((N - l) & (N - 1))]);
+                    const double2 d = csub(P, Q);
+                    p.U[uidx(0, l)] = cscale(cadd(P, Q), 0.5);
+                    p.U[uidx(n1, l)] = make_double2(0.5 * d.y, -0.5 * d.x);
+                } else {
+                    p.U[uidx(k0, l)] = v[s];
+                }
+            }
+            SyncBlock::sync();
+        } else {
+#pragma unroll
+            for (int s = 0; s < V; ++s) p.U[uidx(k0, ts + s * T)] = v[s];
+        }
+    } else if (out) {
 #pragma unroll
         for (int s = 0; s < V; ++s) out[s_tiled(k0, ts + s * T, n1)] = v[s];
     }
 #pragma unroll
-    for (int s = 0; s < V; ++s) v[s] = noAhead ? in[s_tiled(k1, t + s * T, n1)] : sn[s];
-    if (p.fwd) stages_v<V, LOG2N, 0, false>(v, t, twl, X);
+    for (int s = 0; s < V; ++s) v[s] = ZS ? zs : (noAhead ? in[s_tiled(k1, t + s * T, n1)] : sn[s]);
+    if (!ZS && p.fwd) stages_v<V, LOG2N, 0, false>(v, t, twl, X);
     if constexpr (lateY) {
 #pragma unroll
         for (int s = 0; s < V; ++s) y[s] = p.Y[uidx(k1, t + s * T)];
@@ -588,7 +661,10 @@
     }
     if (p.inv) stages_v<V, LOG2N, 0, true>(v, t, twl, X);
     asm volatile("" : "+v"(ts));
-    if (out) {
+    if constexpr (UNP) {
+#pragma unroll
+        for (int s = 0; s < V; ++s) p.U[uidx(k1, ts + s * T)] = v[s];
+    } else if (out) {
 #pragma unroll
         for (int s = 0; s < V; ++s) out[s_tiled(k1, ts + s * T, n1)] = v[s];
     }
diff --git a/semi-blind-image-deblurring-problems-with-tv_amd/csrc/operator.hip b/semi-blind-image-deblurring-problems-with-tv_amd/csrc/operator.hip
--- a/semi-blind-image-deblurring-problems-with-tv_amd/csrc/operator.hip
+++ b/semi-blind-image-deblurring-problems-with-tv_amd/csrc/operator.hip
@@ -21,6 +21,10 @@
     a.dir_fwd = 1;
     a.op = OP_NONE;
     SBTV_TRY(fft_cols_fwd(ctx, fp, in, add, S));
+    if (fp.u_tiled && !fp.generic) {
+        a.U = U;
+        return fft_rows(ctx, fp, S, nullptr, a);
+    }
     SBTV_TRY(fft_rows(ctx, fp, S, S, a));
     return spec_unpack(ctx, fp, S, U);
 }
diff --git a/semi-blind-image-deblurring-problems-with-tv_amd/csrc/salsa.hip b/semi-blind-image-deblurring-problems-with-tv_amd/csrc/salsa.hip
--- a/semi-blind-image-deblurring-problems-with-tv_amd/csrc/salsa.hip
+++ b/semi-blind-image-deblurring-problems-with-tv_amd/csrc/salsa.hip
@@ -9,9 +9,23 @@
 namespace sbtv {
 
 __global__ void salsa_setup_kernel(const double *__restrict__ src, double *__restrict__ par, int npar, int *__restrict__ frozen,
-                                   int batch) {
+                                   int batch, ProxCtrl *__restrict__ ctrl, int thr0, int maxiter, double tol, double tau) {
     for (int i = threadIdx.x; i < npar; i += blockDim.x) par[i] = src[i];
-    for (int b = threadIdx.x; b < batch; b += blockDim.x) frozen[b] = 0;
+    for (int b = threadIdx.x; b < batch; b += blockDim.x) {
+        frozen[b] = 0;
+        ProxCtrl c = ctrl[b];
+        c.k = 0;
+        c.done = 0;
+        c.cur = 0;
+        c.maxiter = maxiter;
+        c.redo = 0;
+        c.f_valid = 0;
+        c.err = 0.0;
+        c.lambda = src[thr0 + b] * 1.0;
+        c.tol = tol;
+        c.tau = tau;
+        ctrl[b] = c;
+    }
 }
 
 __global__ __launch_bounds__(256) void salsa_recover_x_kernel(const double *__restrict__ g, const double *__restrict__ bu,
@@ -65,6 +79,7 @@
     int maxiter = 0, lag = 0, nrb = 0, npb = 0, nl_prox = 0;
     bool want_mse = false, crit2 = false, zero_start = false, direct_last_ok = false, direct_last = false, nox = false,
          spec_ok = false, use_graph = false;
+    bool zs_fast = false, nox_direct = false, bz_fast = false;
     double *xbuf[2] = {nullptr, nullptr}, *u = nullptr, *gb[2] = {nullptr, nullptr}, *bub[2] = {nullptr, nullptr};
     double *par = nullptr, *taps_d = nullptr, *mu_d = nullptr, *thr_d = nullptr;
     double *acc = nullptr, *postp = nullptr, *o4 = nullptr;
@@ -119,6 +134,17 @@
             SBTV_TRY(ws_get_t(ctx, "salsa.g1", cnt, &gb[1]));
         }
         direct_last = direct_last_ok && !nox;
+        static const bool env_direct = [] {
+            const char *e = getenv("SBTV_SALSA_DIRECT_LAST");
+            return !(e && e[0] == '0');
+        }();
+        nox_direct = env_direct && direct_last_ok && nox && maxiter >= 1;
+        static const bool env_zfast = [] {
+            const char *e = getenv("SBTV_SALSA_ZERO_FAST");
+            return !(e && e[0] == '0');
+        }();
+        zs_fast = env_zfast && zero_start && fft_cols_inv_step_ok(op.fp) && !graph_wanted(cnt);
+        bz_fast = env_zfast && !zero_start && fft_cols_inv_step_ok(op.fp) && !graph_wanted(cnt);
         const size_t nt = (size_t)batch * taille * taille;
         npar = nt + 2 * (size_t)batch;
         SBTV_TRY(ws_get_t(ctx, "salsa.par", npar, &par));
@@ -160,7 +186,7 @@
             par_stage[nt + batch + b] = tau[b] / mu[b];
         }
         hipLaunchKernelGGL(salsa_setup_kernel, dim3(1), dim3(256), 0, ctx->stream, (const double *)f_par.at(pd), par, (int)npar,
-                           frozen_d, batch);
+                           frozen_d, batch, pp.ctrl, (int)(nt + batch), opts->TViters, opts->chambolle_tol, opts->chambolle_tau);
         SBTV_HIP(ctx, hipGetLastError());
         return 0;
     }
@@ -185,22 +211,19 @@
     }
 
     int start() {
-        double *x = xbuf[0], *bu = bub[0], *g = gb[0];
+        double *x = xbuf[0], *bu = bub[0];
         if (zero_start) ctx->calls += batch;
         else SBTV_TRY(op_init_x(ctx, op, opts->initialization, yd, xi, x));
-        if (!zero_start) {
-            SBTV_HIP(ctx, hipMemcpyAsync(u, x, sizeof(double) * cnt, hipMemcpyDeviceToDevice, ctx->stream));
-            SBTV_HIP(ctx, hipMemcpyAsync(g, x, sizeof(double) * cnt, hipMemcpyDeviceToDevice, ctx->stream));
-            SBTV_HIP(ctx, hipMemsetAsync(bu, 0, sizeof(double) * cnt, ctx->stream));
-        }
-        SBTV_TRY(prox_reset(ctx, pp, thr_d, 1.0, opts->TViters, opts->chambolle_tol, opts->chambolle_tau, false, nullptr));
+        if (!zero_start && !bz_fast) SBTV_HIP(ctx, hipMemsetAsync(bu, 0, sizeof(double) * cnt, ctx->stream));
         obj_prev.assign(batch, 0.0);
         Collect c{};
         if (zero_start) {
             double *accz = nullptr, *postz = nullptr;
             int nz = 0;
-            SBTV_TRY(salsa_zero_start(ctx, yd, want_mse ? td : nullptr, x, u, bu, P, batch, (double)M * (double)N, &accz, &postz,
-                                      &nz));
+            const bool clear = !zs_fast;
+            if (zs_fast && maxiter < 1) SBTV_HIP(ctx, hipMemsetAsync(x, 0, sizeof(double) * cnt, ctx->stream));
+            SBTV_TRY(salsa_zero_start(ctx, yd, want_mse ? td : nullptr, clear ? x : nullptr, clear ? u : nullptr,
+                                      clear ? bu : nullptr, P, batch, (double)M * (double)N, &accz, &postz, &nz));
             c = Collect{accz, nz, nullptr, 0, postz, nz, nullptr, 0, 0, 0ull, nullptr};
         } else {
             double *tvp = nullptr;
@@ -212,7 +235,7 @@
             a.Y = op.Ys;
             a.acc = acc;
             SBTV_TRY(fft_cols_fwd(ctx, op.fp, x, nullptr, op.S));
-            SBTV_TRY(tvnorm_partials(ctx, u, M, N, batch, &tvp, &ntv));
+            SBTV_TRY(tvnorm_partials(ctx, x, M, N, batch, &tvp, &ntv));
             SBTV_TRY(fft_rows(ctx, op.fp, op.S, nullptr, a));
             if (want_mse) SBTV_TRY(pair_sums(ctx, x, td, P, batch, o4));
             c = Collect{acc, nrb, tvp, ntv, nullptr, 0, nullptr, 0, 0, 0ull, want_mse ? o4 : nullptr};
@@ -284,7 +307,10 @@
         const bool timed = eager && ((outer & 31) == 4 || outer == 12);
         slot_tagged[slot] = tagged;
         slot_spec[slot] = spec;
-        double *xn = (direct_last && outer == maxiter) ? x_out : xbuf[slot];
+        const bool zfirst = zs_fast && outer == 1;
+        const bool bzfirst = bz_fast && outer == 1;
+        const bool last_direct = nox_direct && outer == maxiter;
+        double *xn = ((direct_last || nox_direct) && outer == maxiter) ? x_out : xbuf[slot];
         const double *xprev = xbuf[slot ^ 1];
         SideJob side{};
         if (pend.valid && spec) {
@@ -303,7 +329,8 @@
         ProxPlan pps = pp;
         pps.partials = pp.partials + (size_t)slot * pp.part_stride;
         if (!(zero_start && outer == 1))
-            SBTV_TRY(prox_iterate(ctx, pps, gb[(outer - 1) & 1], opts->TViters, u, outer == (zero_start ? 2 : 1), spec,
+            SBTV_TRY(prox_iterate(ctx, pps, outer == 1 ? xbuf[0] : gb[(outer - 1) & 1], opts->TViters, u,
+                                  outer == (zero_start ? 2 : 1), spec,
                                   spec ? ((outer - 2) * nl_prox) & 1 : 0, side.nblocks ? &side : nullptr));
         if (timed) SBTV_HIP(ctx, hipEventRecord(ev_p1[slot], ctx->stream));
         prox_timed[slot] = timed;
@@ -316,16 +343,20 @@
         a.mu = mu_d;
         a.acc = acc;
         a.frozen = frozen_d;
-        SBTV_TRY(fft_cols_fwd_f(ctx, op.fp, u, bub[(outer - 1) & 1], op.S, frozen_d));
+        a.s_zero = zfirst ? 1 : 0;
+        if (!zfirst) SBTV_TRY(fft_cols_fwd_f(ctx, op.fp, u, bzfirst ? nullptr : bub[(outer - 1) & 1], op.S, frozen_d));
         SBTV_TRY(fft_rows(ctx, op.fp, op.S, op.S, a));
         ColsPost cp;
         cp.u = u;
         cp.bu = bub[outer & 1];
         cp.g = gb[outer & 1];
         if (nox) {
-            cp.bu_in = bub[(outer - 1) & 1];
-            cp.skip_x = 1;
-        }
+            if (!zfirst && !bzfirst) cp.bu_in = bub[(outer - 1) & 1];
+            cp.skip_x = last_direct ? 0 : 1;
+            cp.recover_x = last_direct ? 1 : 0;
+        }
+        cp.zero_in = zfirst ? 1 : 0;
+        cp.zero_bu = bzfirst ? 1 : 0;
         cp.tru = td;
         cp.xprev = crit2 ? xprev : nullptr;
         cp.partials = postp;
@@ -420,6 +451,7 @@
                     SBTV_TRY(stage_out_copy(ctx, out, src, P, flags));
                 continue;
             }
+            if (nox_direct && h_nouter[b] == maxiter) continue;
             const int par = h_nouter[b] & 1;
             const bool dev_direct = direct_last_ok;
             double *dst = dev_direct ? out : xbuf[0] + (size_t)b * P;
diff --git a/semi-blind-image-deblurring-problems-with-tv_amd/csrc/sbtv_internal.h b/semi-blind-image-deblurring-problems-with-tv_amd/csrc/sbtv_internal.h
--- a/semi-blind-image-deblurring-problems-with-tv_amd/csrc/sbtv_internal.h
+++ b/semi-blind-image-deblurring-problems-with-tv_amd/csrc/sbtv_internal.h
@@ -478,6 +478,7 @@
     double *g = nullptr;
     const double *bu_in = nullptr;
     int skip_x = 0;
+    int recover_x = 0;
     const double *tru = nullptr;
     const double *xprev = nullptr;
     double *partials = nullptr;
@@ -488,6 +489,8 @@
     RngArgs mrng = {0ull, 0u, 0u, nullptr};
     ProxArm marm = {nullptr, nullptr, 0, 0.0, 0.0, nullptr};
     MomArgs mom = {nullptr, nullptr, 0, nullptr, 1, 1};
+    int zero_in = 0;
+    int zero_bu = 0;
 };
 int fft_cols_inv_myula(sbtv_ctx *ctx, const FftPlan &pl, const double2 *S, double scale, double *X, const double *prox,
                        const double *Z, const double *sigma2_dev, double gam, double lamb, const RngArgs *rng,
@@ -512,6 +515,8 @@
     double *acc;
     const int *frozen;
     int shared_spec;
+    int s_zero;
+    double2 *U;
 };
 int fft_rows(sbtv_ctx *ctx, const FftPlan &pl, const double2 *Sin, double2 *Sout, const RowsArgs &a);
 int fft_rows_blocks(const FftPlan &pl);
```
